# osqp/OSQP.jl

Hardware: AMD Instinct MI355X
Metric: ADMM iterations/sec (higher is better)
Workload: dtype f64; 1 GPU; rand-1e6; n=1000000, m=1000000, nnz_A=1000000000, nnz_P_full=1000749500, nnz_P_triu=500874750, backend=pcg, check_termination=25, adaptive_rho_interval=50, instances=1

## Files before the change

### osqp.jl_amd/csrc/common.hpp

```cpp
#pragma once
#include <chrono>
#include <hip/hip_runtime.h>
#include <cstdint>
#include <cstdio>
#include <cstdlib>
#include <cstring>
#include <stdexcept>
#include <string>
#include <vector>

#include "../../include/osqp_amd.h"

namespace oq {

struct Error : std::runtime_error {
  int code;
  Error(int c, const std::string &m) : std::runtime_error(m), code(c) {}
};
struct PanelRefused : Error {
  using Error::Error;
};
struct UnsortedColumns : Error {
  UnsortedColumns() : Error(1, "the row indices inside a column of A must ascend (and not repeat)") {}
};
extern thread_local bool g_unsorted_columns;
struct TreeFault : Error {
  TreeFault() : Error(6, "internal: a supernode of the triangular solve waited 200 ms for its children (the solves fall back to one launch per level)") {}
};
void set_last_error(const std::string &m);

#define HIP_CHECK(expr)                                                                             \
  do {                                                                                              \
    hipError_t _e = (expr);                                                                         \
    if (_e != hipSuccess)                                                                           \
      throw oq::Error(6, std::string("HIP error: ") + hipGetErrorString(_e) + " at " + __FILE__ +   \
                             ":" + std::to_string(__LINE__));                                       \
  } while (0)

extern int g_debug_sync;
inline void post_launch(const char *name, hipStream_t s) {
  hipError_t e = hipGetLastError();
  if (e != hipSuccess) throw Error(6, std::string("launch of ") + name + " failed: " + hipGetErrorString(e));
  if (g_debug_sync) {
    fprintf(stderr, "[osqp-amd] %s ... ", name);
    fflush(stderr);
    e = hipStreamSynchronize(s);
    fprintf(stderr, "%s\n", e == hipSuccess ? "ok" : hipGetErrorString(e));
    if (e != hipSuccess) throw Error(6, std::string("kernel ") + name + " failed: " + hipGetErrorString(e));
  }
}
#define OQ_LAUNCH(kern, grid, block, shmem, stream, ...)                    \
  do {                                                                      \
    hipLaunchKernelGGL(kern, grid, block, shmem, stream, __VA_ARGS__);      \
    oq::post_launch(#kern, stream);                                         \
  } while (0)

extern size_t g_device_bytes;
extern size_t g_device_peak;
extern double g_alloc_s, g_free_s;
extern size_t g_cache_bytes;
inline double wall_now() { return std::chrono::duration<double>(std::chrono::steady_clock::now().time_since_epoch()).count(); }

size_t dev_size_class(size_t bytes);
void *dev_alloc(size_t bytes, size_t &granted);
void dev_free(void *p, size_t granted);
void dev_cache_trim();
size_t dev_va_reserved();
struct DevCacheScope {
  DevCacheScope();
  ~DevCacheScope();
  DevCacheScope(const DevCacheScope &) = delete;
  DevCacheScope &operator=(const DevCacheScope &) = delete;
};

template <typename T>
struct DevBuf {
  T *p = nullptr;
  size_t n = 0;
  size_t cap = 0;
  DevBuf() = default;
  explicit DevBuf(size_t count) { alloc(count); }
  DevBuf(const DevBuf &) = delete;
  DevBuf &operator=(const DevBuf &) = delete;
  DevBuf(DevBuf &&o) noexcept : p(o.p), n(o.n), cap(o.cap) { o.p = nullptr; o.n = 0; o.cap = 0; }
  DevBuf &operator=(DevBuf &&o) noexcept {
    if (this != &o) { release(); p = o.p; n = o.n; cap = o.cap; o.p = nullptr; o.n = 0; o.cap = 0; }
    return *this;
  }
  ~DevBuf() { release(); }
  void alloc(size_t count) {
    release();
    n = count;
    p = (T *)dev_alloc((count ? count : 1) * sizeof(T), cap);
  }
  void release() {
    if (p) {
      dev_free(p, cap);
      p = nullptr;
      n = 0;
      cap = 0;
    }
  }
  void zero(hipStream_t s) { HIP_CHECK(hipMemsetAsync(p, 0, (n ? n : 1) * sizeof(T), s)); }
  void upload(const T *h, size_t count, hipStream_t s) {
    if (count) HIP_CHECK(hipMemcpyAsync(p, h, count * sizeof(T), hipMemcpyHostToDevice, s));
  }
  void download(T *h, size_t count, hipStream_t s) const {
    if (count) HIP_CHECK(hipMemcpyAsync(h, p, count * sizeof(T), hipMemcpyDeviceToHost, s));
  }
  T *get() const { return p; }
};

struct DevPanel {
  bool active = false;
  int W = 0, shift = 0, B = 0, Gp = 1, NG = 0, ntiles = 0;
  DevBuf<int> tile_g, tile_r0, tile_r1;
  DevBuf<int> unit_s0, unit_ns;
  DevBuf<uint32_t> slice_base;
  DevBuf<int> slice_len;
  DevBuf<int> slice_rows;
  DevBuf<uint32_t> cellbase;
  DevBuf<double> sval;
  DevBuf<uint16_t> scol;
  bool wide = false;
  DevBuf<uint32_t> scol32;
  DevBuf<double> partial;
  size_t padded = 0;
};

struct DevCsr {
  int rows = 0, cols = 0;
  int64_t nnz = 0;
  DevBuf<int64_t> rowptr;
  DevBuf<int> col;
  DevBuf<double> val;
  DevPanel panel;
  bool compact = false;
  int group = 64;
  double spmv_bytes() const {
    return 12.0 * (double)nnz + 4.0 * ((double)rows + 1.0) + 8.0 * ((double)rows + (double)cols);
  }
};

enum Slot {
  S_PRI = 0, S_PRI_UNS, S_Z, S_AX, S_Z_UNS, S_AX_UNS,
  S_DUA, S_DUA_UNS, S_Q, S_ATY, S_PX, S_Q_UNS, S_ATY_UNS, S_PX_UNS,
  S_XPX, S_QX,
  S_T0, S_T1, S_T2, S_T3, S_T4, S_T5,
  S_COUNT = 32
};

struct Publish {
  double *host_slots = nullptr;
  volatile unsigned long long *host_seq = nullptr;
  unsigned long long seq = 0;
};

constexpr int kBlock = 256;
constexpr int kReduceBlocks = 1024;

inline int blocks_for(int64_t n, int per_block = kBlock) {
  int64_t b = (n + per_block - 1) / per_block;
  if (b < 1) b = 1;
  if (b > 2147483647LL) throw Error(6, "grid too large");
  return (int)b;
}

}
```

### osqp.jl_amd/csrc/panel.hip

```cpp
#include <algorithm>

#include "kernels.hpp"
#include <functional>
#include "devutil.hpp"

namespace oq {

namespace {

constexpr int kThreads = 1024;
#ifndef OQ_SELL_BATCH
#define OQ_SELL_BATCH 16
#endif
constexpr int kBatch = OQ_SELL_BATCH;
constexpr int kWaves = kThreads / 64;
constexpr int kTileRowsMax = 3968;
constexpr int kSortN = 4096;

int env_int(const char *name, int dflt) { const char *e = getenv(name); return e ? atoi(e) : dflt; }
int panel_shift() { return env_int("OSQP_AMD_PANEL_SHIFT", 14); }
int panel_tile_nnz() { return env_int("OSQP_AMD_PANEL_TILE_NNZ", 65536); }

__device__ __forceinline__ int64_t lower_bound_col(const int *__restrict__ col, int64_t s, int64_t e, int target) {
  while (s < e) { int64_t mid = (s + e) >> 1; if (col[mid] < target) s = mid + 1; else e = mid; }
  return s;
}

__global__ __launch_bounds__(kBlock) void k_panel_count(int rows, int B, int shift, const int64_t *__restrict__ rp,
                                                        const int *__restrict__ col, int64_t *__restrict__ cnt,
                                                        uint32_t *__restrict__ cellsrc) {
  const int lane = threadIdx.x & 63;
  const int64_t row = ((int64_t)blockIdx.x * kBlock + threadIdx.x) >> 6;
  if (row >= rows) return;
  const int64_t s = rp[row], e = rp[row + 1];
  for (int b = lane; b < B; b += 64) {
    int64_t lo = lower_bound_col(col, s, e, b << shift);
    int64_t hi = (b + 1 == B) ? e : lower_bound_col(col, s, e, (b + 1) << shift);
    cnt[(size_t)b * rows + row] = hi - lo;
    cellsrc[(size_t)b * rows + row] = (uint32_t)lo;
  }
}

__global__ __launch_bounds__(kBlock) void k_group_count(int rows, int B, int Gp, int64_t gcells, const int64_t *__restrict__ cnt,
                                                        int64_t *__restrict__ gcnt) {
  const int64_t c = (int64_t)blockIdx.x * kBlock + threadIdx.x;
  if (c >= gcells) return;
  const int64_t g = c / rows;
  const int r = (int)(c - g * rows);
  int64_t a = 0;
  for (int b = (int)g * Gp; b < B && b < ((int)g + 1) * Gp; b++) a += cnt[(size_t)b * rows + r];
  gcnt[c] = a;
}
__global__ __launch_bounds__(kBlock) void k_expand_units(int ntiles, int B, int Gp, const int *__restrict__ tile_g,
                                                         const int *__restrict__ tile_r0, const int *__restrict__ tile_r1,
                                                         int *__restrict__ ub, int *__restrict__ u0, int *__restrict__ u1) {
  const int64_t u = (int64_t)blockIdx.x * kBlock + threadIdx.x;
  if (u >= (int64_t)ntiles * Gp) return;
  const int t = (int)(u / Gp), j = (int)(u - (int64_t)t * Gp);
  const int b = tile_g[t] * Gp + j;
  const bool real = b < B;
  ub[u] = real ? b : 0;
  u0[u] = tile_r0[t];
  u1[u] = real ? tile_r1[t] : tile_r0[t];
}

__global__ __launch_bounds__(kBlock) void k_tile_cost(int64_t cells, int64_t cmin, int64_t *__restrict__ cnt) {
  const int64_t c = (int64_t)blockIdx.x * kBlock + threadIdx.x;
  if (c < cells && cnt[c] < cmin) cnt[c] = cmin;
}
__global__ __launch_bounds__(kBlock) void k_tile_starts(int rows, int64_t cells, const int64_t *__restrict__ coff, int64_t budget,
                                                        int64_t *__restrict__ start) {
  const int64_t c = (int64_t)blockIdx.x * kBlock + threadIdx.x;
  if (c >= cells) return;
  const int64_t b = c / rows;
  const int r = (int)(c - b * rows);
  const int64_t *po = coff + b * rows;
  const int64_t base = po[0];
  start[c] = (r == 0 || (po[r - 1] - base) / budget != (po[r] - base) / budget) ? 1 : 0;
}
__global__ __launch_bounds__(kBlock) void k_tile_fill(int rows, int64_t cells, const int64_t *__restrict__ start,
                                                      const int64_t *__restrict__ tid, int *__restrict__ tile_b, int *__restrict__ tile_r0) {
  const int64_t c = (int64_t)blockIdx.x * kBlock + threadIdx.x;
  if (c >= cells || !start[c]) return;
  const int64_t b = c / rows;
  tile_b[tid[c]] = (int)b;
  tile_r0[tid[c]] = (int)(c - b * rows);
}
__global__ __launch_bounds__(kBlock) void k_tile_ends(int rows, int ntiles, const int *__restrict__ tile_b, const int *__restrict__ tile_r0,
                                                      int *__restrict__ tile_r1) {
  const int t = blockIdx.x * kBlock + threadIdx.x;
  if (t >= ntiles) return;
  tile_r1[t] = (t + 1 < ntiles && tile_b[t + 1] == tile_b[t]) ? tile_r0[t + 1] : rows;
}

__device__ void order_tile_rows(uint32_t *key, const int64_t *__restrict__ po, int r0, int nrows, int *nz_rows) {
  if (threadIdx.x == 0) *nz_rows = 0;
  __syncthreads();
  int mine = 0;
  for (int i = threadIdx.x; i < kSortN; i += kThreads) {
    uint32_t k = 0xFFFFFFFFu;
    if (i < nrows) {
      const uint32_t len = (uint32_t)(po[r0 + i + 1] - po[r0 + i]);
      k = ((0x7FFFFu - len) << 12) | (uint32_t)i;
      mine += len > 0;
    }
    key[i] = k;
  }
  if (mine) atomicAdd(nz_rows, mine);
  __syncthreads();
  for (int k = 2; k <= kSortN; k <<= 1)
    for (int j = k >> 1; j > 0; j >>= 1) {
      for (int i = threadIdx.x; i < kSortN; i += kThreads) {
        const int p = i ^ j;
        if (p > i) {
          const uint32_t a = key[i], b = key[p];
          if ((a > b) == ((i & k) == 0)) { key[i] = b; key[p] = a; }
        }
      }
      __syncthreads();
    }
}
__device__ __forceinline__ uint32_t key_len(uint32_t key) { return 0x7FFFFu - (key >> 12); }

__global__ __launch_bounds__(kThreads) void k_tile_measure(int rows, const int *__restrict__ tile_b, const int *__restrict__ tile_r0,
                                                           const int *__restrict__ tile_r1, const int64_t *__restrict__ off,
                                                           int64_t *__restrict__ nslices, int64_t *__restrict__ padded) {
  __shared__ uint32_t key[kSortN];
  __shared__ int nz;
  __shared__ unsigned long long total;
  const int t = blockIdx.x;
  const int r0 = tile_r0[t], nrows = tile_r1[t] - r0;
  if (threadIdx.x == 0) total = 0ULL;
  order_tile_rows(key, off + (size_t)tile_b[t] * rows, r0, nrows, &nz);
  const int ns = (nz + 63) >> 6;
  unsigned long long mine = 0;
  for (int sl = threadIdx.x; sl < ns; sl += kThreads) mine += 64ULL * key_len(key[sl * 64]);
  if (mine) atomicAdd(&total, mine);
  __syncthreads();
  if (threadIdx.x == 0) { nslices[t] = ns; padded[t] = (int64_t)total; }
}
__global__ __launch_bounds__(kThreads) void k_tile_layout(int rows, const int *__restrict__ tile_b, const int *__restrict__ tile_r0,
                                                          const int *__restrict__ tile_r1, const int64_t *__restrict__ off,
                                                          const int64_t *__restrict__ slice0, const int64_t *__restrict__ padded0,
                                                          int *__restrict__ tile_s0, int *__restrict__ tile_ns,
                                                          uint32_t *__restrict__ slice_base, int *__restrict__ slice_len,
                                                          int *__restrict__ slice_rows, uint32_t *__restrict__ cellbase) {
  __shared__ uint32_t key[kSortN];
  __shared__ uint32_t sbase[kSortN / 64 + 1];
  __shared__ int nz;
  const int t = blockIdx.x, b = tile_b[t];
  const int r0 = tile_r0[t], nrows = tile_r1[t] - r0;
  order_tile_rows(key, off + (size_t)b * rows, r0, nrows, &nz);
  const int ns = (nz + 63) >> 6;
  if (threadIdx.x == 0) {
    uint32_t acc = (uint32_t)padded0[t];
    for (int sl = 0; sl < ns; sl++) { sbase[sl] = acc; acc += 64u * key_len(key[sl * 64]); }
    tile_s0[t] = (int)slice0[t];
    tile_ns[t] = ns;
  }
  __syncthreads();
  const int64_t s0 = slice0[t];
  for (int i = threadIdx.x; i < ns * 64; i += kThreads) {
    const int sl = i >> 6, lane = i & 63;
    int row = -1;
    if (i < nz) {
      row = r0 + (int)(key[i] & 4095u);
      cellbase[(size_t)b * rows + row] = sbase[sl] + (uint32_t)lane;
    }
    slice_rows[(size_t)(s0 + sl) * 64 + lane] = row;
    if (lane == 0) { slice_base[s0 + sl] = sbase[sl]; slice_len[s0 + sl] = (int)key_len(key[sl * 64]); }
  }
}

template <typename ColT>
__global__ __launch_bounds__(kBlock) void k_sell_scatter(int rows, int shift, const int64_t *__restrict__ rp, const int *__restrict__ col,
                                                         const double *__restrict__ val, const uint32_t *__restrict__ cellbase,
                                                         ColT *__restrict__ scol, double *__restrict__ sval, int with_cols,
                                                         uint32_t *__restrict__ slot) {
  const int lane = threadIdx.x & 63;
  const int64_t row = ((int64_t)blockIdx.x * kBlock + threadIdx.x) >> 6;
  if (row >= rows) return;
  const int64_t s = rp[row], e = rp[row + 1];
  const int mask = (1 << shift) - 1;
  int carry_b = -1;
  int64_t carry_seg = s;
  for (int64_t k0 = s; k0 < e; k0 += 64) {
    const int64_t k = k0 + lane;
    const bool in = k < e;
    const int c = in ? col[k] : 0x7fffffff;
    const int b = in ? (c >> shift) : 0x7fffffff;
    int bprev = __shfl_up(b, 1, 64);
    if (lane == 0) bprev = carry_b;
    const unsigned long long heads = __ballot(b != bprev);
    const unsigned long long upto = heads & (~0ull >> (63 - lane));
    const int64_t seg = upto ? k0 + (63 - __builtin_clzll(upto)) : carry_seg;
    if (in) {
      const size_t dst = (size_t)cellbase[(size_t)b * rows + row] + (size_t)(k - seg) * 64;
      sval[dst] = val[k];
      if (with_cols) scol[dst] = (ColT)(c & mask);
      if (slot) slot[k] = (uint32_t)dst;
    }
    carry_b = __shfl(b, 63, 64);
    carry_seg = __shfl(seg, 63, 64);
  }
}

constexpr int kFillK = 16;
constexpr int kFillStride = 65;
constexpr int kFillWaves = 4;
template <typename ColT>
__global__ __launch_bounds__(kFillWaves * 64) void k_sell_fill_lds(int rows, int shift, const int *__restrict__ ub, const int *__restrict__ unit_s0,
                                                                 const int *__restrict__ unit_ns, const uint32_t *__restrict__ slice_base,
                                                                 const int *__restrict__ slice_len, const int *__restrict__ slice_rows,
                                                                 const uint32_t *__restrict__ cellsrc, const int64_t *__restrict__ off,
                                                                 const int *__restrict__ col, const double *__restrict__ val,
                                                                 ColT *__restrict__ scol, double *__restrict__ sval, uint32_t *__restrict__ slot,
                                                                 int what) {
  const bool do_cols = what & 1, do_vals = what & 2;
  __shared__ double tv[kFillWaves][kFillK * kFillStride];
  __shared__ uint32_t tc[kFillWaves][kFillK * kFillStride];
  __shared__ int start[kFillWaves][65];
  const int u = blockIdx.x, b = ub[u];
  const int s0 = unit_s0[u], ns = unit_ns[u];
  const int wave = threadIdx.x >> 6, lane = threadIdx.x & 63;
  const int mask = (1 << shift) - 1;
  double *mv = tv[wave];
  uint32_t *mc = tc[wave];
  int *st = start[wave];
  for (int sl = s0 + wave; sl < s0 + ns; sl += kFillWaves) {
    const uint32_t base = slice_base[sl];
    const int L = slice_len[sl];
    const int row = slice_rows[(size_t)sl * 64 + lane];
    uint32_t src = 0;
    int len = 0;
    if (row >= 0) {
      const size_t c = (size_t)b * rows + row;
      src = cellsrc[c];
      len = (int)(off[c + 1] - off[c]);
    }
    for (int k0 = 0; k0 < L; k0 += kFillK) {
      int mine = len - k0;
      mine = mine < 0 ? 0 : (mine > kFillK ? kFillK : mine);
      int incl = mine;
#pragma unroll
      for (int o = 1; o < 64; o <<= 1) { const int t = __shfl_up(incl, o, 64); if (lane >= o) incl += t; }
      const int total = __shfl(incl, 63, 64);
      st[lane] = incl - mine;
      if (lane == 63) st[64] = total;
      __builtin_amdgcn_fence(__ATOMIC_RELEASE, "wavefront");
      __builtin_amdgcn_wave_barrier();
      __builtin_amdgcn_fence(__ATOMIC_ACQUIRE, "wavefront");
      for (int f = lane; f < ((total + 63) & ~63); f += 64) {
        const bool in = f < total;
        int r = 0;
        if (in) {
          int lo = 0, hi = 64;
          while (hi - lo > 1) { const int mid = (lo + hi) >> 1; if (st[mid] <= f) lo = mid; else hi = mid; }
          r = lo;
        }
        const uint32_t rsrc = (uint32_t)__shfl((int)src, r, 64);
        if (in) {
          const int k = f - st[r];
          const size_t g = (size_t)rsrc + (size_t)(k0 + k);
          if (do_vals) mv[k * kFillStride + r] = val[g];
          if (do_cols) {
            mc[k * kFillStride + r] = (uint32_t)(col[g] & mask);
            if (slot) slot[g] = base + (uint32_t)((k0 + k) * 64 + r);
          }
        }
      }
      __builtin_amdgcn_fence(__ATOMIC_RELEASE, "wavefront");
      __builtin_amdgcn_wave_barrier();
      __builtin_amdgcn_fence(__ATOMIC_ACQUIRE, "wavefront");
      const int kend = L - k0 < kFillK ? L - k0 : kFillK;
      for (int k = 0; k < kend; k++) {
        const size_t at = (size_t)base + (size_t)(k0 + k) * 64 + lane;
        const bool in = k < mine;
        if (do_vals) sval[at] = in ? mv[k * kFillStride + lane] : 0.0;
        if (do_cols) scol[at] = in ? (ColT)mc[k * kFillStride + lane] : (ColT)0;
      }
      __builtin_amdgcn_fence(__ATOMIC_RELEASE, "wavefront");
      __builtin_amdgcn_wave_barrier();
    }
  }
}

template <typename ColT, bool kStageX, bool kSquare>
__device__ __forceinline__ void sell_tile(int t, int rows, int cols, int shift, int B, int Gp, const int *__restrict__ tile_g,
                                          const int *__restrict__ tile_r0, const int *__restrict__ tile_r1,
                                          const int *__restrict__ unit_s0, const int *__restrict__ unit_ns,
                                          const uint32_t *__restrict__ slice_base, const int *__restrict__ slice_len,
                                          const int *__restrict__ slice_rows, const ColT *__restrict__ scol,
                                          const double *__restrict__ sval, const double *__restrict__ x, double *__restrict__ partial) {
  extern __shared__ __attribute__((aligned(16))) double lds[];
  const int g = tile_g[t];
  const int W = 1 << shift;
  const int r0 = tile_r0[t], nrows = tile_r1[t] - r0;
  double *xs_lds = lds;
  double *ys = kStageX ? lds + W : lds;
  for (int i = threadIdx.x; i < nrows; i += kThreads) ys[i] = 0.0;
  const int wave = threadIdx.x >> 6, lane = threadIdx.x & 63;
  bool first = true;
  for (int j = 0; j < Gp; j++) {
    const int b = g * Gp + j;
    if (b >= B) break;
    const int s0 = unit_s0[(size_t)t * Gp + j], ns = unit_ns[(size_t)t * Gp + j];
    if (ns == 0) continue;
    const int c0 = b << shift;
    const double *xs = x + c0;
    if (kStageX) {
      if (!first) __syncthreads();
      const int wlen = cols - c0 < W ? cols - c0 : W;
      double2 *xl = reinterpret_cast<double2 *>(xs_lds);
      if (wlen == 16 * kThreads) {
        const double2 *xg = reinterpret_cast<const double2 *>(x + c0);
        double2 v[8];
#pragma unroll
        for (int k = 0; k < 8; k++) v[k] = xg[threadIdx.x + k * kThreads];
#pragma unroll
        for (int k = 0; k < 8; k++) xl[threadIdx.x + k * kThreads] = v[k];
      } else {
        for (int i = threadIdx.x; i < wlen; i += kThreads) xs_lds[i] = x[c0 + i];
      }
      __syncthreads();
      xs = xs_lds;
    } else {
      __syncthreads();
    }
    first = false;
    int sl = s0 + wave;
    size_t nbase = 0;
    int nL = 0, nrow = -1;
    if (sl < s0 + ns) { nbase = (size_t)slice_base[sl]; nL = slice_len[sl]; nrow = slice_rows[(size_t)sl * 64 + lane]; }
    for (; sl < s0 + ns; sl += kWaves) {
      const size_t base = nbase + lane;
      const int L = nL, row = nrow;
      if (sl + kWaves < s0 + ns) {
        nbase = (size_t)slice_base[sl + kWaves]; nL = slice_len[sl + kWaves]; nrow = slice_rows[(size_t)(sl + kWaves) * 64 + lane];
      }
      const double *v = sval + base;
      const ColT *c = scol + base;
      double a0 = 0.0;
      for (int k = 0; k < L; k += kBatch) {
        double cv[kBatch];
        ColT cc[kBatch];
        if (k + kBatch <= L) {
#pragma unroll
          for (int u = 0; u < kBatch; u++) { cv[u] = v[(size_t)(k + u) * 64]; cc[u] = c[(size_t)(k + u) * 64]; }
        } else {
#pragma unroll
          for (int u = 0; u < kBatch; u++) {
            const bool in = k + u < L;
            cv[u] = in ? v[(size_t)(k + u) * 64] : 0.0;
            cc[u] = in ? c[(size_t)(k + u) * 64] : (ColT)0;
          }
        }
#pragma unroll
        for (int u = 0; u < kBatch; u++) a0 += (kSquare ? cv[u] * cv[u] : cv[u]) * xs[cc[u]];
      }
      if (row >= 0) ys[row - r0] += a0;
    }
  }
  __syncthreads();
  double *out = partial + (size_t)g * rows + r0;
  for (int i = threadIdx.x; i < nrows; i += kThreads) out[i] = ys[i];
}
template <typename ColT, bool kStageX, bool kSquare = false>
__global__ __launch_bounds__(kThreads) void k_spmv_sell(int rows, int cols, int shift, int B, int Gp, const int *__restrict__ tile_g,
                                                        const int *__restrict__ tile_r0, const int *__restrict__ tile_r1,
                                                        const int *__restrict__ unit_s0, const int *__restrict__ unit_ns,
                                                        const uint32_t *__restrict__ slice_base, const int *__restrict__ slice_len,
                                                        const int *__restrict__ slice_rows, const ColT *__restrict__ scol,
                                                        const double *__restrict__ sval, const double *__restrict__ x,
                                                        double *__restrict__ partial, const int *__restrict__ skip) {
  if (skip && *skip) return;
  sell_tile<ColT, kStageX, kSquare>(blockIdx.x, rows, cols, shift, B, Gp, tile_g, tile_r0, tile_r1, unit_s0, unit_ns, slice_base, slice_len,
                                    slice_rows, scol, sval, x, partial);
}
struct SellSide {
  int rows, cols, B, Gp, ntiles;
  const int *tile_g, *tile_r0, *tile_r1, *unit_s0, *unit_ns, *slice_len, *slice_rows;
  const uint32_t *slice_base;
  const uint16_t *scol;
  const double *sval;
  double *partial;
};
__global__ __launch_bounds__(kThreads) void k_spmv_sell_pair(SellSide a, SellSide b, int shift, const double *__restrict__ x,
                                                             const int *__restrict__ skip) {
  if (skip && *skip) return;
  const bool first = (int)blockIdx.x < a.ntiles;
  const SellSide &m = first ? a : b;
  sell_tile<uint16_t, true, false>(first ? (int)blockIdx.x : (int)blockIdx.x - a.ntiles, m.rows, m.cols, shift, m.B, m.Gp, m.tile_g, m.tile_r0,
                                   m.tile_r1, m.unit_s0, m.unit_ns, m.slice_base, m.slice_len, m.slice_rows, m.scol, m.sval, x, m.partial);
}

__device__ __forceinline__ void panel_reduce_rows(int vb, int vg, int rows, int B, const double *__restrict__ partial, double *__restrict__ y,
                                                  const double *__restrict__ rscale, double beta, double gamma,
                                                  const double *__restrict__ v, const SpmvExtra &ex) {
  double dot = 0.0, mx = 0.0, num = 0.0, den = 0.0;
  for (int i = vb * kBlock + threadIdx.x; i < rows; i += vg * kBlock) {
    double acc = 0.0;
    int b = 0;
    for (; b + 8 <= B; b += 8) {
      double t[8];
#pragma unroll
      for (int u = 0; u < 8; u++) t[u] = partial[(size_t)(b + u) * rows + i];
#pragma unroll
      for (int u = 0; u < 8; u++) acc += t[u];
    }
    if (b + 4 <= B) {
      double t[4];
#pragma unroll
      for (int u = 0; u < 4; u++) t[u] = partial[(size_t)(b + u) * rows + i];
#pragma unroll
      for (int u = 0; u < 4; u++) acc += t[u];
      b += 4;
    }
    for (; b < B; b++) acc += partial[(size_t)b * rows + i];
    if (ex.y2) ex.y2[i] = ex.s2[i] * acc;
    if (rscale) acc *= rscale[i];
    if (beta != 0.0) acc += beta * y[i];
    if (v) acc += gamma * v[i];
    y[i] = acc;
    if (ex.dotv) dot += ex.dotv[i] * acc;
    if (ex.absmax_slot) mx = nanmax(mx, fabs(acc));
    if (ex.e2_partials) {
      const double d = ex.e2_x1[i] - ex.e2_x0[i], m1 = ex.e2_m1[i];
      num += d * (acc - m1);
      den += d * (m1 - ex.e2_m0[i]);
    }
  }
  if (ex.e2_partials) {
    num = block_sum(num);
    den = block_sum(den);
    if (threadIdx.x == 0) { ex.e2_partials[vb] = num; ex.e2_partials[kReduceBlocks + vb] = den; }
    if (vb == 0)
      for (int t = vg + threadIdx.x; t < kReduceBlocks; t += kBlock) { ex.e2_partials[t] = 0.0; ex.e2_partials[kReduceBlocks + t] = 0.0; }
  }
  if (ex.dot_partials) {
    dot = block_sum(dot);
    if (threadIdx.x == 0) ex.dot_partials[vb] = dot;
    if (vb == 0)
      for (int t = vg + threadIdx.x; t < kReduceBlocks; t += kBlock) ex.dot_partials[t] = 0.0;
  }
  if (ex.absmax_slot) {
    mx = block_max(mx);
    if (threadIdx.x == 0) atomic_max_nonneg(ex.absmax_slot, mx);
  }
}
__global__ __launch_bounds__(kBlock) void k_panel_reduce(int rows, int B, const double *__restrict__ partial, double *__restrict__ y,
                                                         const double *__restrict__ rscale, double beta, double gamma,
                                                         const double *__restrict__ v, SpmvExtra ex, const int *__restrict__ skip) {
  if (skip && *skip) return;
  panel_reduce_rows(blockIdx.x, gridDim.x, rows, B, partial, y, rscale, beta, gamma, v, ex);
}
struct ReduceSide {
  int rows, B, grid;
  const double *partial;
  double *y;
  double gamma;
  const double *v;
  SpmvExtra ex;
};
__global__ __launch_bounds__(kBlock) void k_panel_reduce_pair(ReduceSide a, ReduceSide b, const int *__restrict__ skip) {
  if (skip && *skip) return;
  const bool first = (int)blockIdx.x < a.grid;
  const ReduceSide &m = first ? a : b;
  panel_reduce_rows(first ? (int)blockIdx.x : (int)blockIdx.x - a.grid, m.grid, m.rows, m.B, m.partial, m.y, nullptr, 0.0, m.gamma, m.v, m.ex);
}

template <typename ColT, int kOp>
__global__ __launch_bounds__(kThreads) void k_sell_visit(int rows, int shift, int B, int Gp, const int *__restrict__ tile_g,
                                                         const int *__restrict__ tile_r0, const int *__restrict__ tile_r1,
                                                         const int *__restrict__ unit_s0, const int *__restrict__ unit_ns,
                                                         const uint32_t *__restrict__ slice_base, const int *__restrict__ slice_len,
                                                         const int *__restrict__ slice_rows, const ColT *__restrict__ scol,
                                                         double *__restrict__ sval, const double *__restrict__ r, const double *__restrict__ c,
                                                         int order, double scalar, int row0, double *__restrict__ out) {
  __shared__ double ys[kOp == 1 ? kTileRowsMax : 1];
  const int t = blockIdx.x, g = tile_g[t];
  const int r0 = tile_r0[t], nrows = tile_r1[t] - r0;
  const int wave = threadIdx.x >> 6, lane = threadIdx.x & 63;
  if (kOp == 1) for (int i = threadIdx.x; i < nrows; i += kThreads) ys[i] = 0.0;
  for (int j = 0; j < Gp; j++) {
    const int b = g * Gp + j;
    if (b >= B) break;
    const int s0 = unit_s0[(size_t)t * Gp + j], ns = unit_ns[(size_t)t * Gp + j];
    if (kOp == 1) __syncthreads();
    const int c0 = b << shift;
    for (int sl = s0 + wave; sl < s0 + ns; sl += kWaves) {
      const size_t base = (size_t)slice_base[sl] + lane;
      const int L = slice_len[sl];
      const int row = slice_rows[(size_t)sl * 64 + lane];
      if (row < 0) continue;
      double mx = 0.0;
      for (int k = 0; k < L; k++) {
        const size_t at = base + (size_t)k * 64;
        double v = sval[at];
        if (kOp == 0) {
          if (r) {
            const int col = c0 + (int)scol[at];
            double a, bb;
            if (order == 1) { const int gi = row + row0; const int lo = col < gi ? col : gi, hi = col < gi ? gi : col; a = c[lo]; bb = c[hi]; }
            else if (order == 2) { a = c[col]; bb = r[row]; }
            else { a = r[row]; bb = c[col]; }
            v = (v * a) * bb;
          }
          if (scalar != 1.0) v *= scalar;
          if (v != 0.0 || sval[at] != 0.0) sval[at] = v;
        } else if (kOp == 1) {
          mx = fmax(mx, fabs(v));
        } else {
          if (c0 + (int)scol[at] == row + row0 && v != 0.0) out[row] = v;
        }
      }
      if (kOp == 1) ys[row - r0] = fmax(ys[row - r0], mx);
    }
  }
  if (kOp == 1) {
    __syncthreads();
    double *o = out + (size_t)g * rows + r0;
    for (int i = threadIdx.x; i < nrows; i += kThreads) o[i] = ys[i];
  }
}
template <typename ColT>
__global__ __launch_bounds__(kThreads) void k_sell_scale_norm(int rows, int cols, int shift, int B, int Gp, const int *__restrict__ tile_g,
                                                              const int *__restrict__ tile_r0, const int *__restrict__ tile_r1,
                                                              const int *__restrict__ unit_s0, const int *__restrict__ unit_ns,
                                                              const uint32_t *__restrict__ slice_base, const int *__restrict__ slice_len,
                                                              const int *__restrict__ slice_rows, const ColT *__restrict__ scol,
                                                              double *__restrict__ sval, const double *__restrict__ r,
                                                              const double *__restrict__ c, int order, double pre, int row0,
                                                              double *__restrict__ partial) {
  extern __shared__ __attribute__((aligned(16))) double lds[];
  const int t = blockIdx.x, g = tile_g[t];
  const int W = 1 << shift;
  const int r0 = tile_r0[t], nrows = tile_r1[t] - r0;
  double *cs = lds, *ys = lds + W;
  for (int i = threadIdx.x; i < nrows; i += kThreads) ys[i] = 0.0;
  const int wave = threadIdx.x >> 6, lane = threadIdx.x & 63;
  const double *rv = order == 1 ? c + row0 : r;
  bool first = true;
  for (int j = 0; j < Gp; j++) {
    const int b = g * Gp + j;
    if (b >= B) break;
    const int s0 = unit_s0[(size_t)t * Gp + j], ns = unit_ns[(size_t)t * Gp + j];
    if (ns == 0) continue;
    const int c0 = b << shift;
    if (!first) __syncthreads();
    const int wlen = cols - c0 < W ? cols - c0 : W;
    if (wlen == 16 * kThreads) {
      const double2 *xg = reinterpret_cast<const double2 *>(c + c0);
      double2 *xl = reinterpret_cast<double2 *>(cs);
      double2 v[8];
#pragma unroll
      for (int k = 0; k < 8; k++) v[k] = xg[threadIdx.x + k * kThreads];
#pragma unroll
      for (int k = 0; k < 8; k++) xl[threadIdx.x + k * kThreads] = v[k];
    } else {
      for (int i = threadIdx.x; i < wlen; i += kThreads) cs[i] = c[c0 + i];
    }
    __syncthreads();
    first = false;
    int sl = s0 + wave;
    size_t nbase = 0;
    int nL = 0, nrow = -1;
    double nrs = 1.0;
    if (sl < s0 + ns) {
      nbase = (size_t)slice_base[sl]; nL = slice_len[sl]; nrow = slice_rows[(size_t)sl * 64 + lane];
      nrs = nrow >= 0 ? rv[nrow] : 1.0;
    }
    for (; sl < s0 + ns; sl += kWaves) {
      const size_t base = nbase + lane;
      const int L = nL, row = nrow;
      const double rs = nrs;
      if (sl + kWaves < s0 + ns) {
        nbase = (size_t)slice_base[sl + kWaves]; nL = slice_len[sl + kWaves]; nrow = slice_rows[(size_t)(sl + kWaves) * 64 + lane];
        nrs = nrow >= 0 ? rv[nrow] : 1.0;
      }
      double *v = sval + base;
      const ColT *cc_ = scol + base;
      const int grow = row + row0 - c0;
      double mx = 0.0;
      for (int k = 0; k < L; k += kBatch) {
        double cv[kBatch];
        ColT cc[kBatch];
        const bool full = k + kBatch <= L;
        if (full) {
#pragma unroll
          for (int u = 0; u < kBatch; u++) { cv[u] = v[(size_t)(k + u) * 64]; cc[u] = cc_[(size_t)(k + u) * 64]; }
        } else {
#pragma unroll
          for (int u = 0; u < kBatch; u++) {
            const bool in = k + u < L;
            cv[u] = in ? v[(size_t)(k + u) * 64] : 0.0;
            cc[u] = in ? cc_[(size_t)(k + u) * 64] : (ColT)0;
          }
        }
#pragma unroll
        for (int u = 0; u < kBatch; u++) {
          double x = cv[u];
          if (pre != 1.0) x *= pre;
          const double cf = cs[cc[u]];
          if (order == 1) { const bool below = (int)cc[u] < grow; x = (x * (below ? cf : rs)) * (below ? rs : cf); }
          else if (order == 2) x = (x * cf) * rs;
          else x = (x * rs) * cf;
          cv[u] = x;
          mx = fmax(mx, fabs(x));
        }
        if (row >= 0) {
          if (full) {
#pragma unroll
            for (int u = 0; u < kBatch; u++) v[(size_t)(k + u) * 64] = cv[u];
          } else {
#pragma unroll
            for (int u = 0; u < kBatch; u++) if (k + u < L) v[(size_t)(k + u) * 64] = cv[u];
          }
        }
      }
      if (row >= 0) ys[row - r0] = fmax(ys[row - r0], mx);
    }
  }
  __syncthreads();
  double *out = partial + (size_t)g * rows + r0;
  for (int i = threadIdx.x; i < nrows; i += kThreads) out[i] = ys[i];
}
__global__ __launch_bounds__(kBlock) void k_panel_reduce_max(int rows, int NG, const double *__restrict__ partial, double *__restrict__ out,
                                                             int accumulate) {
  const int i = blockIdx.x * kBlock + threadIdx.x;
  if (i >= rows) return;
  double m = 0.0;
  for (int g = 0; g < NG; g++) m = fmax(m, partial[(size_t)g * rows + i]);
  out[i] = accumulate ? fmax(out[i], m) : m;
}
__global__ __launch_bounds__(kBlock) void k_sell_slot_of_pos(int rows, int shift, const int64_t *__restrict__ rp, const int *__restrict__ col,
                                                             const uint32_t *__restrict__ cellbase, uint32_t *__restrict__ slot) {
  const int lane = threadIdx.x & 63;
  const int64_t row = ((int64_t)blockIdx.x * kBlock + threadIdx.x) >> 6;
  if (row >= rows) return;
  const int64_t s = rp[row], e = rp[row + 1];
  for (int64_t k = s + lane; k < e; k += 64) {
    const int b = col[k] >> shift;
    const int64_t seg = lower_bound_col(col, s, k + 1, b << shift);
    slot[k] = (uint32_t)((size_t)cellbase[(size_t)b * rows + row] + (size_t)(k - seg) * 64);
  }
}

size_t spmv_lds_bytes(int shift) { return (sizeof(double) << shift) + sizeof(double) * kTileRowsMax; }

int64_t read_i64(const int64_t *dev, hipStream_t s) {
  int64_t v = 0;
  HIP_CHECK(hipMemcpyAsync(&v, dev, sizeof(int64_t), hipMemcpyDeviceToHost, s));
  HIP_CHECK(hipStreamSynchronize(s));
  return v;
}

}

static int panel_group_size(const DevCsr &M, int B) {
  const int want = env_int("OSQP_AMD_PANEL_GROUP", 0);
  if (want > 0) return std::min(want, B);
  if ((double)M.nnz / (4.0 * (double)panel_tile_nnz()) >= 1024.0) return std::min(4, B);
  return 1;
}

static int wide_shift(const DevCsr &M) {
  if (const int forced = env_int("OSQP_AMD_WIDE_SHIFT", 0)) return forced;
  for (int sh = 18; sh <= 20; sh++) {
    const int Bw = (M.cols + (1 << sh) - 1) >> sh;
    if (Bw < 4) return 0;
    if ((double)M.nnz / ((double)M.rows * Bw) >= 3.5) return sh;
  }
  return 0;
}
static int panel_mode(const DevCsr &M) {
  const int shift = panel_shift();
  if (const char *e = getenv("OSQP_AMD_PANEL")) {
    if (atoi(e) == 0) return 0;
    if (atoi(e) == 2) return M.cols > (1 << shift) ? 1 : 0;
    if (atoi(e) == 3) return M.cols > (1 << shift) ? 2 : 0;
  }
  if (M.nnz < 2000000 || M.nnz >= 4000000000LL) return 0;
  const int B = (M.cols + (1 << shift) - 1) >> shift;
  if (B >= 2) {
    const int Gp = panel_group_size(M, B), NG = (B + Gp - 1) / Gp;
    if ((double)M.nnz / ((double)M.rows * NG) >= 4.0 && (double)M.nnz / ((double)M.rows * B) >= 1.5) return 1;
  }
  return wide_shift(M) ? 2 : 0;
}

bool panel_wanted(const DevCsr &M) { return panel_mode(M) != 0; }

void panel_fill(DevCsr &M, bool with_cols, hipStream_t s, uint32_t *slot) {
  DevPanel &P = M.panel;
  if (P.wide)
    OQ_LAUNCH(k_sell_scatter<uint32_t>, dim3(blocks_for((int64_t)M.rows * 64)), dim3(kBlock), 0, s, M.rows, P.shift, M.rowptr.get(),
              M.col.get(), M.val.get(), P.cellbase.get(), P.scol32.get(), P.sval.get(), with_cols ? 1 : 0, slot);
  else
    OQ_LAUNCH(k_sell_scatter<uint16_t>, dim3(blocks_for((int64_t)M.rows * 64)), dim3(kBlock), 0, s, M.rows, P.shift, M.rowptr.get(),
              M.col.get(), M.val.get(), P.cellbase.get(), P.scol.get(), P.sval.get(), with_cols ? 1 : 0, slot);
}

void panel_build(DevCsr &M, hipStream_t s, uint32_t *slot, bool will_compact, const std::function<void()> &after_cols) {
  DevPanel &P = M.panel;
  P.wide = panel_mode(M) == 2;
  P.shift = P.wide ? (wide_shift(M) ? wide_shift(M) : 18) : panel_shift(); P.W = 1 << P.shift;
  if (!P.wide && P.shift > 15) throw PanelRefused(6, "panel width above 2^15 columns is not supported (16-bit local column ids, LDS size)");
  P.B = (M.cols + P.W - 1) >> P.shift;
  const int64_t cells = (int64_t)P.B * M.rows;
  DevBuf<int64_t> cnt((size_t)cells + 1), off((size_t)cells + 1);
  DevBuf<uint32_t> cellsrc((size_t)cells);
  OQ_LAUNCH(k_panel_count, dim3(blocks_for((int64_t)M.rows * 64)), dim3(kBlock), 0, s, M.rows, P.B, P.shift, M.rowptr.get(),
            M.col.get(), cnt.get(), cellsrc.get());
  exclusive_scan(cnt.get(), off.get(), cells, s);
  P.Gp = panel_group_size(M, P.B);
  P.NG = (P.B + P.Gp - 1) / P.Gp;
  const int64_t gcells = (int64_t)P.NG * M.rows;
  DevBuf<int64_t> gcnt((size_t)gcells + 1), tid((size_t)gcells + 1);
  OQ_LAUNCH(k_group_count, dim3(blocks_for(gcells)), dim3(kBlock), 0, s, M.rows, P.B, P.Gp, gcells, cnt.get(), gcnt.get());
  cnt.release();
  int64_t tile_nnz = panel_tile_nnz();
  if (!getenv("OSQP_AMD_PANEL_TILE_NNZ") && P.Gp == 1) {
    int dev = 0, cus = 256;
    if (hipGetDevice(&dev) == hipSuccess) (void)hipDeviceGetAttribute(&cus, hipDeviceAttributeMultiprocessorCount, dev);
    if ((double)M.nnz / (double)tile_nnz < (double)cus)
      tile_nnz = std::max<int64_t>(32768, std::min<int64_t>(tile_nnz, (int64_t)((double)M.nnz / (0.85 * (double)cus))));
  }
  const int64_t budget = std::max<int64_t>(tile_nnz * P.Gp, kTileRowsMax);
  const int64_t cmin = (budget + kTileRowsMax - 1) / kTileRowsMax;
  OQ_LAUNCH(k_tile_cost, dim3(blocks_for(gcells)), dim3(kBlock), 0, s, gcells, cmin, gcnt.get());
  exclusive_scan(gcnt.get(), tid.get(), gcells, s);
  OQ_LAUNCH(k_tile_starts, dim3(blocks_for(gcells)), dim3(kBlock), 0, s, M.rows, gcells, tid.get(), budget, gcnt.get());
  exclusive_scan(gcnt.get(), tid.get(), gcells, s);
  const int64_t ntiles = read_i64(tid.get() + gcells, s);
  if (ntiles <= 0 || ntiles * P.Gp >= 2147483647LL) throw PanelRefused(6, "panel layout: bad tile count");
  P.ntiles = (int)ntiles;
  P.tile_g.alloc((size_t)ntiles); P.tile_r0.alloc((size_t)ntiles); P.tile_r1.alloc((size_t)ntiles);
  OQ_LAUNCH(k_tile_fill, dim3(blocks_for(gcells)), dim3(kBlock), 0, s, M.rows, gcells, gcnt.get(), tid.get(), P.tile_g.get(), P.tile_r0.get());
  OQ_LAUNCH(k_tile_ends, dim3(blocks_for(ntiles)), dim3(kBlock), 0, s, M.rows, P.ntiles, P.tile_g.get(), P.tile_r0.get(), P.tile_r1.get());
  const int64_t nunits = ntiles * P.Gp;
  DevBuf<int> ub((size_t)nunits), u0((size_t)nunits), u1((size_t)nunits);
  OQ_LAUNCH(k_expand_units, dim3(blocks_for(nunits)), dim3(kBlock), 0, s, P.ntiles, P.B, P.Gp, P.tile_g.get(), P.tile_r0.get(),
            P.tile_r1.get(), ub.get(), u0.get(), u1.get());
  HIP_CHECK(hipStreamSynchronize(s));
  gcnt.release(); tid.release();
  DevBuf<int64_t> nsl((size_t)nunits + 1), pad((size_t)nunits + 1), slice0((size_t)nunits + 1), padded0((size_t)nunits + 1);
  OQ_LAUNCH(k_tile_measure, dim3((unsigned)nunits), dim3(kThreads), 0, s, M.rows, ub.get(), u0.get(), u1.get(), off.get(), nsl.get(), pad.get());
  exclusive_scan(nsl.get(), slice0.get(), nunits, s);
  exclusive_scan(pad.get(), padded0.get(), nunits, s);
  const int64_t nslices = read_i64(slice0.get() + nunits, s), padded = read_i64(padded0.get() + nunits, s);
  if (padded >= 4294967295LL) throw PanelRefused(6, "sliced-ELL copy exceeds 2^32 entries");
  if (!getenv("OSQP_AMD_PANEL") && (double)padded > 1.5 * (double)M.nnz) throw PanelRefused(6, "sliced-ELL copy would be mostly padding");
  P.padded = (size_t)padded;
  P.unit_s0.alloc((size_t)nunits); P.unit_ns.alloc((size_t)nunits);
  P.slice_base.alloc((size_t)nslices); P.slice_len.alloc((size_t)nslices); P.slice_rows.alloc((size_t)nslices * 64);
  P.cellbase.alloc((size_t)cells); P.cellbase.zero(s);
  OQ_LAUNCH(k_tile_layout, dim3((unsigned)nunits), dim3(kThreads), 0, s, M.rows, ub.get(), u0.get(), u1.get(), off.get(), slice0.get(),
            padded0.get(), P.unit_s0.get(), P.unit_ns.get(), P.slice_base.get(), P.slice_len.get(), P.slice_rows.get(), P.cellbase.get());
  P.partial.alloc((size_t)gcells);
  P.partial.zero(s);
  static const bool lds_fill = !(getenv("OSQP_AMD_SELL_FILL") && atoi(getenv("OSQP_AMD_SELL_FILL")) == 0);
  auto fill = [&](int what) {
    if (P.wide)
      OQ_LAUNCH(k_sell_fill_lds<uint32_t>, dim3((unsigned)nunits), dim3(kFillWaves * 64), 0, s, M.rows, P.shift, ub.get(), P.unit_s0.get(),
                P.unit_ns.get(), P.slice_base.get(), P.slice_len.get(), P.slice_rows.get(), cellsrc.get(), off.get(), M.col.get(), M.val.get(),
                P.scol32.get(), P.sval.get(), slot, what);
    else
      OQ_LAUNCH(k_sell_fill_lds<uint16_t>, dim3((unsigned)nunits), dim3(kFillWaves * 64), 0, s, M.rows, P.shift, ub.get(), P.unit_s0.get(),
                P.unit_ns.get(), P.slice_base.get(), P.slice_len.get(), P.slice_rows.get(), cellsrc.get(), off.get(), M.col.get(), M.val.get(),
                P.scol.get(), P.sval.get(), slot, what);
  };
  if (!lds_fill) {
    P.sval.alloc((size_t)padded);
    P.sval.zero(s);
    if (P.wide) { P.scol32.alloc((size_t)padded); P.scol32.zero(s); }
    else { P.scol.alloc((size_t)padded); P.scol.zero(s); }
    panel_fill(M, true, s, slot);
  } else if (will_compact && !P.wide) {
    P.scol.alloc((size_t)padded);
    fill(1);
    HIP_CHECK(hipStreamSynchronize(s));
    M.col.release();
    if (after_cols) after_cols();
    P.sval.alloc((size_t)padded);
    fill(2);
  } else {
    P.sval.alloc((size_t)padded);
    if (P.wide) P.scol32.alloc((size_t)padded); else P.scol.alloc((size_t)padded);
    fill(3);
  }
  HIP_CHECK(hipStreamSynchronize(s));
  if (!P.wide)
    HIP_CHECK(hipFuncSetAttribute((const void *)k_spmv_sell<uint16_t, true>, hipFuncAttributeMaxDynamicSharedMemorySize,
                                  (int)spmv_lds_bytes(P.shift)));
  P.active = true;
}

static int reduce_grid(int rows) { return std::min(blocks_for(rows), kReduceBlocks); }

void spmv_panel(const DevCsr &M, const double *x, double *y, const double *rscale, double beta, double gamma, const double *v,
                hipStream_t s, const SpmvExtra *extra) {
  const DevPanel &P = M.panel;
  const SpmvExtra ex = extra ? *extra : SpmvExtra();
  if (P.wide)
    OQ_LAUNCH((k_spmv_sell<uint32_t, false>), dim3(P.ntiles), dim3(kThreads), sizeof(double) * kTileRowsMax, s, M.rows, M.cols, P.shift, P.B,
              P.Gp, P.tile_g.get(), P.tile_r0.get(), P.tile_r1.get(), P.unit_s0.get(), P.unit_ns.get(), P.slice_base.get(),
              P.slice_len.get(), P.slice_rows.get(), P.scol32.get(), P.sval.get(), x, P.partial.get(), g_skip);
  else
    OQ_LAUNCH((k_spmv_sell<uint16_t, true>), dim3(P.ntiles), dim3(kThreads), spmv_lds_bytes(P.shift), s, M.rows, M.cols, P.shift, P.B,
              P.Gp, P.tile_g.get(), P.tile_r0.get(), P.tile_r1.get(), P.unit_s0.get(), P.unit_ns.get(), P.slice_base.get(),
              P.slice_len.get(), P.slice_rows.get(), P.scol.get(), P.sval.get(), x, P.partial.get(), g_skip);
  OQ_LAUNCH(k_panel_reduce, dim3(reduce_grid(M.rows)), dim3(kBlock), 0, s, M.rows, P.NG, P.partial.get(), y, rscale, beta, gamma, v, ex, g_skip);
}

bool spmv_pair_ok(const DevCsr &Ma, const DevCsr &Mb) {
  const DevPanel &A = Ma.panel, &B = Mb.panel;
  static const bool enabled = !(getenv("OSQP_AMD_SPMV_PAIR") && atoi(getenv("OSQP_AMD_SPMV_PAIR")) == 0);
  return enabled && A.active && B.active && !A.wide && !B.wide && A.shift == B.shift && Ma.cols == Mb.cols && A.ntiles + B.ntiles <= 2048;
}
void spmv_pair(const DevCsr &Ma, const DevCsr &Mb, const double *x, double *ya, const SpmvExtra *extra_a, double *yb, double gamma_b,
               const double *vb, hipStream_t s) {
  auto side = [](const DevCsr &M) {
    const DevPanel &P = M.panel;
    SellSide t;
    t.rows = M.rows; t.cols = M.cols; t.B = P.B; t.Gp = P.Gp; t.ntiles = P.ntiles;
    t.tile_g = P.tile_g.get(); t.tile_r0 = P.tile_r0.get(); t.tile_r1 = P.tile_r1.get(); t.unit_s0 = P.unit_s0.get(); t.unit_ns = P.unit_ns.get();
    t.slice_len = P.slice_len.get(); t.slice_rows = P.slice_rows.get(); t.slice_base = P.slice_base.get(); t.scol = P.scol.get();
    t.sval = P.sval.get(); t.partial = P.partial.get();
    return t;
  };
  const DevPanel &A = Ma.panel, &B = Mb.panel;
  static bool attr_set = false;
  if (!attr_set) {
    HIP_CHECK(hipFuncSetAttribute((const void *)k_spmv_sell_pair, hipFuncAttributeMaxDynamicSharedMemorySize, (int)spmv_lds_bytes(A.shift)));
    attr_set = true;
  }
  OQ_LAUNCH(k_spmv_sell_pair, dim3(A.ntiles + B.ntiles), dim3(kThreads), spmv_lds_bytes(A.shift), s, side(Ma), side(Mb), A.shift, x, g_skip);
  ReduceSide ra{Ma.rows, A.NG, reduce_grid(Ma.rows), A.partial.get(), ya, 0.0, nullptr, extra_a ? *extra_a : SpmvExtra()};
  ReduceSide rb{Mb.rows, B.NG, reduce_grid(Mb.rows), B.partial.get(), yb, gamma_b, vb, SpmvExtra()};
  OQ_LAUNCH(k_panel_reduce_pair, dim3(ra.grid + rb.grid), dim3(kBlock), 0, s, ra, rb, g_skip);
}

#define OQ_SELL_VISIT(OP, ...)                                                                                                              \
  do {                                                                                                                                      \
    if (P.wide) OQ_LAUNCH((k_sell_visit<uint32_t, OP>), dim3(P.ntiles), dim3(kThreads), 0, s, M.rows, P.shift, P.B, P.Gp, P.tile_g.get(),    \
                          P.tile_r0.get(), P.tile_r1.get(), P.unit_s0.get(), P.unit_ns.get(), P.slice_base.get(), P.slice_len.get(),        \
                          P.slice_rows.get(), P.scol32.get(), P.sval.get(), __VA_ARGS__);                                                    \
    else OQ_LAUNCH((k_sell_visit<uint16_t, OP>), dim3(P.ntiles), dim3(kThreads), 0, s, M.rows, P.shift, P.B, P.Gp, P.tile_g.get(),           \
                   P.tile_r0.get(), P.tile_r1.get(), P.unit_s0.get(), P.unit_ns.get(), P.slice_base.get(), P.slice_len.get(),               \
                   P.slice_rows.get(), P.scol.get(), P.sval.get(), __VA_ARGS__);                                                             \
  } while (0)

void panel_row_absmax(const DevCsr &M, double *out, bool accumulate, hipStream_t s) {
  const DevPanel &P = M.panel;
  OQ_SELL_VISIT(1, (const double *)nullptr, (const double *)nullptr, 0, 1.0, 0, P.partial.get());
  OQ_LAUNCH(k_panel_reduce_max, dim3(blocks_for(M.rows)), dim3(kBlock), 0, s, M.rows, P.NG, P.partial.get(), out, (int)accumulate);
}
void panel_scale(DevCsr &M, const double *r, const double *c, int order, double scalar, hipStream_t s, int row0) {
  const DevPanel &P = M.panel;
  OQ_SELL_VISIT(0, r, c, order, scalar, row0, (double *)nullptr);
}
void panel_scale_norm(DevCsr &M, const double *r, const double *c, int order, double pre, int row0, double *norm, hipStream_t s) {
  const DevPanel &P = M.panel;
  if (P.wide) throw Error(6, "internal: the fused scaling pass needs LDS-staged panels");
  HIP_CHECK(hipFuncSetAttribute((const void *)k_sell_scale_norm<uint16_t>, hipFuncAttributeMaxDynamicSharedMemorySize,
                                (int)spmv_lds_bytes(P.shift)));
  OQ_LAUNCH((k_sell_scale_norm<uint16_t>), dim3(P.ntiles), dim3(kThreads), spmv_lds_bytes(P.shift), s, M.rows, M.cols, P.shift, P.B, P.Gp,
            P.tile_g.get(), P.tile_r0.get(), P.tile_r1.get(), P.unit_s0.get(), P.unit_ns.get(), P.slice_base.get(), P.slice_len.get(),
            P.slice_rows.get(), P.scol.get(), P.sval.get(), r, c, order, pre, row0, P.partial.get());
  OQ_LAUNCH(k_panel_reduce_max, dim3(blocks_for(M.rows)), dim3(kBlock), 0, s, M.rows, P.NG, P.partial.get(), norm, 0);
}
void panel_diag(const DevCsr &M, double *diag, int row0, hipStream_t s) {
  const DevPanel &P = M.panel;
  HIP_CHECK(hipMemsetAsync(diag, 0, sizeof(double) * (size_t)M.rows, s));
  OQ_SELL_VISIT(2, (const double *)nullptr, (const double *)nullptr, 0, 1.0, row0, diag);
}
#undef OQ_SELL_VISIT
void spmv_panel_squared(const DevCsr &M, const double *x, double *y, double gamma, const double *v, hipStream_t s) {
  const DevPanel &P = M.panel;
  HIP_CHECK(hipFuncSetAttribute((const void *)k_spmv_sell<uint16_t, true, true>, hipFuncAttributeMaxDynamicSharedMemorySize,
                                (int)spmv_lds_bytes(P.shift)));
  OQ_LAUNCH((k_spmv_sell<uint16_t, true, true>), dim3(P.ntiles), dim3(kThreads), spmv_lds_bytes(P.shift), s, M.rows, M.cols, P.shift, P.B,
            P.Gp, P.tile_g.get(), P.tile_r0.get(), P.tile_r1.get(), P.unit_s0.get(), P.unit_ns.get(), P.slice_base.get(),
            P.slice_len.get(), P.slice_rows.get(), P.scol.get(), P.sval.get(), x, P.partial.get(), (const int *)nullptr);
  OQ_LAUNCH(k_panel_reduce, dim3(reduce_grid(M.rows)), dim3(kBlock), 0, s, M.rows, P.NG, P.partial.get(), y, (const double *)nullptr, 0.0, gamma, v,
            SpmvExtra(), (const int *)nullptr);
}
void panel_slot_of_pos(const DevCsr &M, uint32_t *slot, hipStream_t s) {
  const DevPanel &P = M.panel;
  OQ_LAUNCH(k_sell_slot_of_pos, dim3(blocks_for((int64_t)M.rows * 64)), dim3(kBlock), 0, s, M.rows, P.shift, M.rowptr.get(), M.col.get(),
            P.cellbase.get(), slot);
}
bool panel_can_compact(const DevCsr &M) { return M.panel.active && !M.panel.wide; }
void panel_compact(DevCsr &M) {
  M.col.release();
  M.val.release();
  M.panel.cellbase.release();
  M.compact = true;
}

}
```

Baseline: 83.39 iterations/s.

## Compact SELL slices by dropping padding lanes per column in aligned groups

Changes the SELL panel layout so that each column of a slice only stores as many lanes as the rows still active there, rounded up to an alignment group (default 64, set through an env var). It packs row length and local row index into one per-lane word, adds per-slice column-start tables, and updates the measure, layout, scatter, fill and SpMV kernels to compute offsets with ballot/popcount. The aim is to cut padded zero storage and memory traffic in SpMV for rows of uneven length. In exchange it adds per-element offset arithmetic, less regular access patterns and extra setup tables.

```diff
diff --git a/osqp.jl_amd/csrc/common.hpp b/osqp.jl_amd/csrc/common.hpp
--- a/osqp.jl_amd/csrc/common.hpp
+++ b/osqp.jl_amd/csrc/common.hpp
@@ -118,8 +118,10 @@
   DevBuf<int> unit_s0, unit_ns;
   DevBuf<uint32_t> slice_base;
   DevBuf<int> slice_len;
-  DevBuf<int> slice_rows;
+  DevBuf<uint32_t> slice_lanes;
+  int align = 64;
   DevBuf<uint32_t> cellbase;
+  DevBuf<uint32_t> slice_tab, colstart;
   DevBuf<double> sval;
   DevBuf<uint16_t> scol;
   bool wide = false;
diff --git a/osqp.jl_amd/csrc/panel.hip b/osqp.jl_amd/csrc/panel.hip
--- a/osqp.jl_amd/csrc/panel.hip
+++ b/osqp.jl_amd/csrc/panel.hip
@@ -2,6 +2,7 @@
 
 #include "kernels.hpp"
 #include <functional>
+#include <type_traits>
 #include "devutil.hpp"
 
 namespace oq {
@@ -20,6 +21,12 @@
 int env_int(const char *name, int dflt) { const char *e = getenv(name); return e ? atoi(e) : dflt; }
 int panel_shift() { return env_int("OSQP_AMD_PANEL_SHIFT", 14); }
 int panel_tile_nnz() { return env_int("OSQP_AMD_PANEL_TILE_NNZ", 65536); }
+constexpr int kSellAlign = 64;
+constexpr int kSlack = 64;
+int sell_align() {
+  const int g = env_int("OSQP_AMD_SELL_ALIGN", kSellAlign);
+  return (g >= 1 && g <= 64 && (g & (g - 1)) == 0) ? g : kSellAlign;
+}
 
 __device__ __forceinline__ int64_t lower_bound_col(const int *__restrict__ col, int64_t s, int64_t e, int target) {
   while (s < e) { int64_t mid = (s + e) >> 1; if (col[mid] < target) s = mid + 1; else e = mid; }
@@ -121,60 +128,99 @@
     }
 }
 __device__ __forceinline__ uint32_t key_len(uint32_t key) { return 0x7FFFFu - (key >> 12); }
-
-__global__ __launch_bounds__(kThreads) void k_tile_measure(int rows, const int *__restrict__ tile_b, const int *__restrict__ tile_r0,
+__device__ __forceinline__ int lane_len(uint32_t w) { return (int)(w >> 12); }
+__device__ __forceinline__ int lane_row(uint32_t w, int r0) { return w ? r0 + (int)(w & 4095u) : -1; }
+template <typename T>
+__device__ __forceinline__ T &slice_at(T *base, uint32_t idx) {
+  return *reinterpret_cast<T *>(reinterpret_cast<char *>(const_cast<typename std::remove_const<T>::type *>(base)) + (size_t)(idx * (uint32_t)sizeof(T)));
+}
+__device__ __forceinline__ int wave_id() { return __builtin_amdgcn_readfirstlane((int)(threadIdx.x >> 6)); }
+__device__ __forceinline__ uint32_t column_lanes(bool in, int gm) {
+  return (uint32_t)((__popcll(__ballot(in)) + gm) & ~gm);
+}
+
+__global__ __launch_bounds__(kThreads) void k_tile_measure(int rows, int G, const int *__restrict__ tile_b, const int *__restrict__ tile_r0,
                                                            const int *__restrict__ tile_r1, const int64_t *__restrict__ off,
-                                                           int64_t *__restrict__ nslices, int64_t *__restrict__ padded) {
+                                                           int64_t *__restrict__ nslices, int64_t *__restrict__ padded,
+                                                           int64_t *__restrict__ lensum) {
   __shared__ uint32_t key[kSortN];
   __shared__ int nz;
-  __shared__ unsigned long long total;
+  __shared__ unsigned long long total, total64;
   const int t = blockIdx.x;
   const int r0 = tile_r0[t], nrows = tile_r1[t] - r0;
-  if (threadIdx.x == 0) total = 0ULL;
+  if (threadIdx.x == 0) { total = 0ULL; total64 = 0ULL; }
   order_tile_rows(key, off + (size_t)tile_b[t] * rows, r0, nrows, &nz);
   const int ns = (nz + 63) >> 6;
-  unsigned long long mine = 0;
-  for (int sl = threadIdx.x; sl < ns; sl += kThreads) mine += 64ULL * key_len(key[sl * 64]);
+  unsigned long long mine = 0, mine64 = 0;
+  for (int i = threadIdx.x * G; i < nz; i += kThreads * G) {
+    mine += (unsigned long long)G * key_len(key[i]);
+    if ((i & 63) == 0) mine64 += key_len(key[i]);
+  }
   if (mine) atomicAdd(&total, mine);
+  if (mine64) atomicAdd(&total64, mine64);
   __syncthreads();
-  if (threadIdx.x == 0) { nslices[t] = ns; padded[t] = (int64_t)total; }
-}
-__global__ __launch_bounds__(kThreads) void k_tile_layout(int rows, const int *__restrict__ tile_b, const int *__restrict__ tile_r0,
+  if (threadIdx.x == 0) { nslices[t] = ns; padded[t] = (int64_t)total; lensum[t] = (int64_t)total64; }
+}
+__global__ __launch_bounds__(kThreads) void k_tile_layout(int rows, int G, const int *__restrict__ tile_b, const int *__restrict__ tile_r0,
                                                           const int *__restrict__ tile_r1, const int64_t *__restrict__ off,
                                                           const int64_t *__restrict__ slice0, const int64_t *__restrict__ padded0,
-                                                          int *__restrict__ tile_s0, int *__restrict__ tile_ns,
-                                                          uint32_t *__restrict__ slice_base, int *__restrict__ slice_len,
-                                                          int *__restrict__ slice_rows, uint32_t *__restrict__ cellbase) {
+                                                          const int64_t *__restrict__ lensum0, int *__restrict__ tile_s0,
+                                                          int *__restrict__ tile_ns, uint32_t *__restrict__ slice_base,
+                                                          int *__restrict__ slice_len, uint32_t *__restrict__ slice_lanes,
+                                                          uint32_t *__restrict__ cellbase, uint32_t *__restrict__ slice_tab,
+                                                          uint32_t *__restrict__ colstart) {
   __shared__ uint32_t key[kSortN];
-  __shared__ uint32_t sbase[kSortN / 64 + 1];
+  __shared__ uint32_t sbase[kSortN / 64 + 1], stab[kSortN / 64 + 1];
   __shared__ int nz;
   const int t = blockIdx.x, b = tile_b[t];
   const int r0 = tile_r0[t], nrows = tile_r1[t] - r0;
+  for (int i = threadIdx.x; i <= kSortN / 64; i += kThreads) sbase[i] = 0u;
   order_tile_rows(key, off + (size_t)b * rows, r0, nrows, &nz);
   const int ns = (nz + 63) >> 6;
+  for (int i = threadIdx.x * G; i < nz; i += kThreads * G) atomicAdd(&sbase[i >> 6], (uint32_t)G * key_len(key[i]));
+  __syncthreads();
   if (threadIdx.x == 0) {
-    uint32_t acc = (uint32_t)padded0[t];
-    for (int sl = 0; sl < ns; sl++) { sbase[sl] = acc; acc += 64u * key_len(key[sl * 64]); }
+    uint32_t acc = (uint32_t)padded0[t], tab = (uint32_t)lensum0[t];
+    for (int sl = 0; sl < ns; sl++) {
+      const uint32_t size = sbase[sl];
+      sbase[sl] = acc; acc += size;
+      stab[sl] = tab; tab += key_len(key[sl * 64]);
+    }
     tile_s0[t] = (int)slice0[t];
     tile_ns[t] = ns;
   }
   __syncthreads();
   const int64_t s0 = slice0[t];
+  const int gm = G - 1;
   for (int i = threadIdx.x; i < ns * 64; i += kThreads) {
     const int sl = i >> 6, lane = i & 63;
-    int row = -1;
+    uint32_t w = 0u;
     if (i < nz) {
-      row = r0 + (int)(key[i] & 4095u);
-      cellbase[(size_t)b * rows + row] = sbase[sl] + (uint32_t)lane;
-    }
-    slice_rows[(size_t)(s0 + sl) * 64 + lane] = row;
-    if (lane == 0) { slice_base[s0 + sl] = sbase[sl]; slice_len[s0 + sl] = (int)key_len(key[sl * 64]); }
-  }
-}
-
+      const uint32_t local = key[i] & 4095u;
+      w = (key_len(key[i]) << 12) | local;
+      cellbase[(size_t)b * rows + r0 + (int)local] = (uint32_t)(s0 + sl) * 64u + (uint32_t)lane;
+    }
+    slice_lanes[(size_t)(s0 + sl) * 64 + lane] = w;
+    const int len = lane_len(w), L = (int)key_len(key[sl * 64]);
+    if (lane == 0) { slice_base[s0 + sl] = sbase[sl]; slice_len[s0 + sl] = L; slice_tab[s0 + sl] = stab[sl]; }
+    uint32_t start = 0u;
+    for (int k = 0; k < L; k++) {
+      if (lane == 0) colstart[(size_t)stab[sl] + k] = start;
+      start += column_lanes(k < len, gm);
+    }
+  }
+}
+
+__device__ __forceinline__ size_t cell_slot(uint32_t cell, int64_t j, const uint32_t *__restrict__ slice_base,
+                                            const uint32_t *__restrict__ slice_tab, const uint32_t *__restrict__ colstart) {
+  const uint32_t sl = cell >> 6;
+  return (size_t)slice_base[sl] + (size_t)colstart[(size_t)slice_tab[sl] + (size_t)j] + (size_t)(cell & 63u);
+}
 template <typename ColT>
 __global__ __launch_bounds__(kBlock) void k_sell_scatter(int rows, int shift, const int64_t *__restrict__ rp, const int *__restrict__ col,
                                                          const double *__restrict__ val, const uint32_t *__restrict__ cellbase,
+                                                         const uint32_t *__restrict__ slice_base, const uint32_t *__restrict__ slice_tab,
+                                                         const uint32_t *__restrict__ colstart,
                                                          ColT *__restrict__ scol, double *__restrict__ sval, int with_cols,
                                                          uint32_t *__restrict__ slot) {
   const int lane = threadIdx.x & 63;
@@ -195,7 +241,7 @@
     const unsigned long long upto = heads & (~0ull >> (63 - lane));
     const int64_t seg = upto ? k0 + (63 - __builtin_clzll(upto)) : carry_seg;
     if (in) {
-      const size_t dst = (size_t)cellbase[(size_t)b * rows + row] + (size_t)(k - seg) * 64;
+      const size_t dst = cell_slot(cellbase[(size_t)b * rows + row], k - seg, slice_base, slice_tab, colstart);
       sval[dst] = val[k];
       if (with_cols) scol[dst] = (ColT)(c & mask);
       if (slot) slot[k] = (uint32_t)dst;
@@ -209,10 +255,11 @@
 constexpr int kFillStride = 65;
 constexpr int kFillWaves = 4;
 template <typename ColT>
-__global__ __launch_bounds__(kFillWaves * 64) void k_sell_fill_lds(int rows, int shift, const int *__restrict__ ub, const int *__restrict__ unit_s0,
+__global__ __launch_bounds__(kFillWaves * 64) void k_sell_fill_lds(int rows, int shift, int gm, const int *__restrict__ ub, const int *__restrict__ u0,
+                                                                 const int *__restrict__ unit_s0,
                                                                  const int *__restrict__ unit_ns, const uint32_t *__restrict__ slice_base,
-                                                                 const int *__restrict__ slice_len, const int *__restrict__ slice_rows,
-                                                                 const uint32_t *__restrict__ cellsrc, const int64_t *__restrict__ off,
+                                                                 const int *__restrict__ slice_len, const uint32_t *__restrict__ slice_lanes,
+                                                                 const uint32_t *__restrict__ cellsrc,
                                                                  const int *__restrict__ col, const double *__restrict__ val,
                                                                  ColT *__restrict__ scol, double *__restrict__ sval, uint32_t *__restrict__ slot,
                                                                  int what) {
@@ -220,7 +267,7 @@
   __shared__ double tv[kFillWaves][kFillK * kFillStride];
   __shared__ uint32_t tc[kFillWaves][kFillK * kFillStride];
   __shared__ int start[kFillWaves][65];
-  const int u = blockIdx.x, b = ub[u];
+  const int u = blockIdx.x, b = ub[u], r0 = u0[u];
   const int s0 = unit_s0[u], ns = unit_ns[u];
   const int wave = threadIdx.x >> 6, lane = threadIdx.x & 63;
   const int mask = (1 << shift) - 1;
@@ -230,17 +277,18 @@
   for (int sl = s0 + wave; sl < s0 + ns; sl += kFillWaves) {
     const uint32_t base = slice_base[sl];
     const int L = slice_len[sl];
-    const int row = slice_rows[(size_t)sl * 64 + lane];
-    uint32_t src = 0;
-    int len = 0;
-    if (row >= 0) {
-      const size_t c = (size_t)b * rows + row;
-      src = cellsrc[c];
-      len = (int)(off[c + 1] - off[c]);
-    }
+    const uint32_t w = slice_lanes[(size_t)sl * 64 + lane];
+    const int row = lane_row(w, r0), len = lane_len(w);
+    const uint32_t src = row >= 0 ? cellsrc[(size_t)b * rows + row] : 0u;
+    uint32_t cstart = 0u;
     for (int k0 = 0; k0 < L; k0 += kFillK) {
       int mine = len - k0;
       mine = mine < 0 ? 0 : (mine > kFillK ? kFillK : mine);
+      uint32_t kstart = 0u;
+      for (int k = 0; k < kFillK; k++) {
+        if (lane == k) kstart = cstart;
+        cstart += column_lanes(k < mine, gm);
+      }
       int incl = mine;
 #pragma unroll
       for (int o = 1; o < 64; o <<= 1) { const int t = __shfl_up(incl, o, 64); if (lane >= o) incl += t; }
@@ -263,21 +311,22 @@
           const int k = f - st[r];
           const size_t g = (size_t)rsrc + (size_t)(k0 + k);
           if (do_vals) mv[k * kFillStride + r] = val[g];
-          if (do_cols) {
-            mc[k * kFillStride + r] = (uint32_t)(col[g] & mask);
-            if (slot) slot[g] = base + (uint32_t)((k0 + k) * 64 + r);
-          }
+          if (do_cols) mc[k * kFillStride + r] = (uint32_t)(col[g] & mask);
         }
+        const uint32_t ks = (uint32_t)__shfl((int)kstart, in ? f - st[r] : 0, 64);
+        if (in && do_cols && slot) slot[(size_t)rsrc + (size_t)(k0 + f - st[r])] = base + ks + (uint32_t)r;
       }
       __builtin_amdgcn_fence(__ATOMIC_RELEASE, "wavefront");
       __builtin_amdgcn_wave_barrier();
       __builtin_amdgcn_fence(__ATOMIC_ACQUIRE, "wavefront");
       const int kend = L - k0 < kFillK ? L - k0 : kFillK;
       for (int k = 0; k < kend; k++) {
-        const size_t at = (size_t)base + (size_t)(k0 + k) * 64 + lane;
+        const size_t at = (size_t)base + (size_t)__shfl((int)kstart, k, 64) + lane;
         const bool in = k < mine;
-        if (do_vals) sval[at] = in ? mv[k * kFillStride + lane] : 0.0;
-        if (do_cols) scol[at] = in ? (ColT)mc[k * kFillStride + lane] : (ColT)0;
+        if (lane < (int)column_lanes(in, gm)) {
+          if (do_vals) sval[at] = in ? mv[k * kFillStride + lane] : 0.0;
+          if (do_cols) scol[at] = in ? (ColT)mc[k * kFillStride + lane] : (ColT)0;
+        }
       }
       __builtin_amdgcn_fence(__ATOMIC_RELEASE, "wavefront");
       __builtin_amdgcn_wave_barrier();
@@ -286,11 +335,11 @@
 }
 
 template <typename ColT, bool kStageX, bool kSquare>
-__device__ __forceinline__ void sell_tile(int t, int rows, int cols, int shift, int B, int Gp, const int *__restrict__ tile_g,
+__device__ __forceinline__ void sell_tile(int t, int rows, int cols, int shift, int gm, int B, int Gp, const int *__restrict__ tile_g,
                                           const int *__restrict__ tile_r0, const int *__restrict__ tile_r1,
                                           const int *__restrict__ unit_s0, const int *__restrict__ unit_ns,
                                           const uint32_t *__restrict__ slice_base, const int *__restrict__ slice_len,
-                                          const int *__restrict__ slice_rows, const ColT *__restrict__ scol,
+                                          const uint32_t *__restrict__ slice_lanes, const ColT *__restrict__ scol,
                                           const double *__restrict__ sval, const double *__restrict__ x, double *__restrict__ partial) {
   extern __shared__ __attribute__((aligned(16))) double lds[];
   const int g = tile_g[t];
@@ -299,7 +348,7 @@
   double *xs_lds = lds;
   double *ys = kStageX ? lds + W : lds;
   for (int i = threadIdx.x; i < nrows; i += kThreads) ys[i] = 0.0;
-  const int wave = threadIdx.x >> 6, lane = threadIdx.x & 63;
+  const int wave = wave_id(), lane = threadIdx.x & 63;
   bool first = true;
   for (int j = 0; j < Gp; j++) {
     const int b = g * Gp + j;
@@ -330,35 +379,43 @@
     first = false;
     int sl = s0 + wave;
     size_t nbase = 0;
-    int nL = 0, nrow = -1;
-    if (sl < s0 + ns) { nbase = (size_t)slice_base[sl]; nL = slice_len[sl]; nrow = slice_rows[(size_t)sl * 64 + lane]; }
+    int nL = 0;
+    uint32_t nw = 0u;
+    if (sl < s0 + ns) { nbase = (size_t)slice_base[sl]; nL = slice_len[sl]; nw = slice_lanes[(size_t)sl * 64 + lane]; }
     for (; sl < s0 + ns; sl += kWaves) {
-      const size_t base = nbase + lane;
-      const int L = nL, row = nrow;
+      const double *v = sval + nbase;
+      const ColT *c = scol + nbase;
+      const int L = nL, len = lane_len(nw), row = (int)(nw & 4095u);
       if (sl + kWaves < s0 + ns) {
-        nbase = (size_t)slice_base[sl + kWaves]; nL = slice_len[sl + kWaves]; nrow = slice_rows[(size_t)(sl + kWaves) * 64 + lane];
+        nbase = (size_t)slice_base[sl + kWaves]; nL = slice_len[sl + kWaves]; nw = slice_lanes[(size_t)(sl + kWaves) * 64 + lane];
       }
-      const double *v = sval + base;
-      const ColT *c = scol + base;
       double a0 = 0.0;
+      uint32_t start = (uint32_t)lane;
       for (int k = 0; k < L; k += kBatch) {
         double cv[kBatch];
         ColT cc[kBatch];
+        uint32_t at[kBatch];
+#pragma unroll
+        for (int u = 0; u < kBatch; u++) { at[u] = start; start += column_lanes(k + u < len, gm); }
         if (k + kBatch <= L) {
 #pragma unroll
-          for (int u = 0; u < kBatch; u++) { cv[u] = v[(size_t)(k + u) * 64]; cc[u] = c[(size_t)(k + u) * 64]; }
+          for (int u = 0; u < kBatch; u++) { cv[u] = slice_at(v, at[u]); cc[u] = slice_at(c, at[u]); }
         } else {
 #pragma unroll
           for (int u = 0; u < kBatch; u++) {
             const bool in = k + u < L;
-            cv[u] = in ? v[(size_t)(k + u) * 64] : 0.0;
-            cc[u] = in ? c[(size_t)(k + u) * 64] : (ColT)0;
+            cv[u] = in ? slice_at(v, at[u]) : 0.0;
+            cc[u] = in ? slice_at(c, at[u]) : (ColT)0;
           }
         }
 #pragma unroll
-        for (int u = 0; u < kBatch; u++) a0 += (kSquare ? cv[u] * cv[u] : cv[u]) * xs[cc[u]];
+        for (int u = 0; u < kBatch; u++) {
+          const bool mine = k + u < len;
+          const double val = mine ? cv[u] : 0.0;
+          a0 += (kSquare ? val * val : val) * xs[mine ? cc[u] : (ColT)0];
+        }
       }
-      if (row >= 0) ys[row - r0] += a0;
+      if (len > 0) ys[row] += a0;
     }
   }
   __syncthreads();
@@ -366,21 +423,21 @@
   for (int i = threadIdx.x; i < nrows; i += kThreads) out[i] = ys[i];
 }
 template <typename ColT, bool kStageX, bool kSquare = false>
-__global__ __launch_bounds__(kThreads) void k_spmv_sell(int rows, int cols, int shift, int B, int Gp, const int *__restrict__ tile_g,
+__global__ __launch_bounds__(kThreads) void k_spmv_sell(int rows, int cols, int shift, int gm, int B, int Gp, const int *__restrict__ tile_g,
                                                         const int *__restrict__ tile_r0, const int *__restrict__ tile_r1,
                                                         const int *__restrict__ unit_s0, const int *__restrict__ unit_ns,
                                                         const uint32_t *__restrict__ slice_base, const int *__restrict__ slice_len,
-                                                        const int *__restrict__ slice_rows, const ColT *__restrict__ scol,
+                                                        const uint32_t *__restrict__ slice_lanes, const ColT *__restrict__ scol,
                                                         const double *__restrict__ sval, const double *__restrict__ x,
                                                         double *__restrict__ partial, const int *__restrict__ skip) {
   if (skip && *skip) return;
-  sell_tile<ColT, kStageX, kSquare>(blockIdx.x, rows, cols, shift, B, Gp, tile_g, tile_r0, tile_r1, unit_s0, unit_ns, slice_base, slice_len,
-                                    slice_rows, scol, sval, x, partial);
+  sell_tile<ColT, kStageX, kSquare>(blockIdx.x, rows, cols, shift, gm, B, Gp, tile_g, tile_r0, tile_r1, unit_s0, unit_ns, slice_base, slice_len,
+                                    slice_lanes, scol, sval, x, partial);
 }
 struct SellSide {
-  int rows, cols, B, Gp, ntiles;
-  const int *tile_g, *tile_r0, *tile_r1, *unit_s0, *unit_ns, *slice_len, *slice_rows;
-  const uint32_t *slice_base;
+  int rows, cols, B, Gp, ntiles, gm;
+  const int *tile_g, *tile_r0, *tile_r1, *unit_s0, *unit_ns, *slice_len;
+  const uint32_t *slice_base, *slice_lanes;
   const uint16_t *scol;
   const double *sval;
   double *partial;
@@ -390,8 +447,8 @@
   if (skip && *skip) return;
   const bool first = (int)blockIdx.x < a.ntiles;
   const SellSide &m = first ? a : b;
-  sell_tile<uint16_t, true, false>(first ? (int)blockIdx.x : (int)blockIdx.x - a.ntiles, m.rows, m.cols, shift, m.B, m.Gp, m.tile_g, m.tile_r0,
-                                   m.tile_r1, m.unit_s0, m.unit_ns, m.slice_base, m.slice_len, m.slice_rows, m.scol, m.sval, x, m.partial);
+  sell_tile<uint16_t, true, false>(first ? (int)blockIdx.x : (int)blockIdx.x - a.ntiles, m.rows, m.cols, shift, m.gm, m.B, m.Gp, m.tile_g, m.tile_r0,
+                                   m.tile_r1, m.unit_s0, m.unit_ns, m.slice_base, m.slice_len, m.slice_lanes, m.scol, m.sval, x, m.partial);
 }
 
 __device__ __forceinline__ void panel_reduce_rows(int vb, int vg, int rows, int B, const double *__restrict__ partial, double *__restrict__ y,
@@ -470,11 +527,11 @@
 }
 
 template <typename ColT, int kOp>
-__global__ __launch_bounds__(kThreads) void k_sell_visit(int rows, int shift, int B, int Gp, const int *__restrict__ tile_g,
+__global__ __launch_bounds__(kThreads) void k_sell_visit(int rows, int shift, int gm, int B, int Gp, const int *__restrict__ tile_g,
                                                          const int *__restrict__ tile_r0, const int *__restrict__ tile_r1,
                                                          const int *__restrict__ unit_s0, const int *__restrict__ unit_ns,
                                                          const uint32_t *__restrict__ slice_base, const int *__restrict__ slice_len,
-                                                         const int *__restrict__ slice_rows, const ColT *__restrict__ scol,
+                                                         const uint32_t *__restrict__ slice_lanes, const ColT *__restrict__ scol,
                                                          double *__restrict__ sval, const double *__restrict__ r, const double *__restrict__ c,
                                                          int order, double scalar, int row0, double *__restrict__ out) {
   __shared__ double ys[kOp == 1 ? kTileRowsMax : 1];
@@ -491,11 +548,14 @@
     for (int sl = s0 + wave; sl < s0 + ns; sl += kWaves) {
       const size_t base = (size_t)slice_base[sl] + lane;
       const int L = slice_len[sl];
-      const int row = slice_rows[(size_t)sl * 64 + lane];
-      if (row < 0) continue;
+      const uint32_t w = slice_lanes[(size_t)sl * 64 + lane];
+      const int row = lane_row(w, r0), len = lane_len(w);
       double mx = 0.0;
+      uint32_t start = 0u;
       for (int k = 0; k < L; k++) {
-        const size_t at = base + (size_t)k * 64;
+        const size_t at = base + start;
+        start += column_lanes(k < len, gm);
+        if (k >= len) continue;
         double v = sval[at];
         if (kOp == 0) {
           if (r) {
@@ -514,7 +574,7 @@
           if (c0 + (int)scol[at] == row + row0 && v != 0.0) out[row] = v;
         }
       }
-      if (kOp == 1) ys[row - r0] = fmax(ys[row - r0], mx);
+      if (kOp == 1 && len > 0) ys[row - r0] = fmax(ys[row - r0], mx);
     }
   }
   if (kOp == 1) {
@@ -524,11 +584,11 @@
   }
 }
 template <typename ColT>
-__global__ __launch_bounds__(kThreads) void k_sell_scale_norm(int rows, int cols, int shift, int B, int Gp, const int *__restrict__ tile_g,
+__global__ __launch_bounds__(kThreads) void k_sell_scale_norm(int rows, int cols, int shift, int gm, int B, int Gp, const int *__restrict__ tile_g,
                                                               const int *__restrict__ tile_r0, const int *__restrict__ tile_r1,
                                                               const int *__restrict__ unit_s0, const int *__restrict__ unit_ns,
                                                               const uint32_t *__restrict__ slice_base, const int *__restrict__ slice_len,
-                                                              const int *__restrict__ slice_rows, const ColT *__restrict__ scol,
+                                                              const uint32_t *__restrict__ slice_lanes, const ColT *__restrict__ scol,
                                                               double *__restrict__ sval, const double *__restrict__ r,
                                                               const double *__restrict__ c, int order, double pre, int row0,
                                                               double *__restrict__ partial) {
@@ -538,7 +598,7 @@
   const int r0 = tile_r0[t], nrows = tile_r1[t] - r0;
   double *cs = lds, *ys = lds + W;
   for (int i = threadIdx.x; i < nrows; i += kThreads) ys[i] = 0.0;
-  const int wave = threadIdx.x >> 6, lane = threadIdx.x & 63;
+  const int wave = wave_id(), lane = threadIdx.x & 63;
   const double *rv = order == 1 ? c + row0 : r;
   bool first = true;
   for (int j = 0; j < Gp; j++) {
@@ -566,39 +626,46 @@
     size_t nbase = 0;
     int nL = 0, nrow = -1;
     double nrs = 1.0;
+    uint32_t nw = 0u;
     if (sl < s0 + ns) {
-      nbase = (size_t)slice_base[sl]; nL = slice_len[sl]; nrow = slice_rows[(size_t)sl * 64 + lane];
+      nbase = (size_t)slice_base[sl]; nL = slice_len[sl]; nw = slice_lanes[(size_t)sl * 64 + lane];
+      nrow = lane_row(nw, r0);
       nrs = nrow >= 0 ? rv[nrow] : 1.0;
     }
     for (; sl < s0 + ns; sl += kWaves) {
-      const size_t base = nbase + lane;
-      const int L = nL, row = nrow;
+      double *v = sval + nbase;
+      const ColT *cc_ = scol + nbase;
+      const int L = nL, row = nrow, len = lane_len(nw);
       const double rs = nrs;
       if (sl + kWaves < s0 + ns) {
-        nbase = (size_t)slice_base[sl + kWaves]; nL = slice_len[sl + kWaves]; nrow = slice_rows[(size_t)(sl + kWaves) * 64 + lane];
+        nbase = (size_t)slice_base[sl + kWaves]; nL = slice_len[sl + kWaves]; nw = slice_lanes[(size_t)(sl + kWaves) * 64 + lane];
+        nrow = lane_row(nw, r0);
         nrs = nrow >= 0 ? rv[nrow] : 1.0;
       }
-      double *v = sval + base;
-      const ColT *cc_ = scol + base;
       const int grow = row + row0 - c0;
       double mx = 0.0;
+      uint32_t start = (uint32_t)lane;
       for (int k = 0; k < L; k += kBatch) {
         double cv[kBatch];
         ColT cc[kBatch];
+        uint32_t at[kBatch];
+#pragma unroll
+        for (int u = 0; u < kBatch; u++) { at[u] = start; start += column_lanes(k + u < len, gm); }
         const bool full = k + kBatch <= L;
         if (full) {
 #pragma unroll
-          for (int u = 0; u < kBatch; u++) { cv[u] = v[(size_t)(k + u) * 64]; cc[u] = cc_[(size_t)(k + u) * 64]; }
+          for (int u = 0; u < kBatch; u++) { cv[u] = slice_at(v, at[u]); cc[u] = slice_at(cc_, at[u]); }
         } else {
 #pragma unroll
           for (int u = 0; u < kBatch; u++) {
             const bool in = k + u < L;
-            cv[u] = in ? v[(size_t)(k + u) * 64] : 0.0;
-            cc[u] = in ? cc_[(size_t)(k + u) * 64] : (ColT)0;
+            cv[u] = in ? slice_at(v, at[u]) : 0.0;
+            cc[u] = in ? slice_at(cc_, at[u]) : (ColT)0;
           }
         }
 #pragma unroll
         for (int u = 0; u < kBatch; u++) {
+          if (k + u >= len) { cv[u] = 0.0; cc[u] = (ColT)0; }
           double x = cv[u];
           if (pre != 1.0) x *= pre;
           const double cf = cs[cc[u]];
@@ -608,15 +675,8 @@
           cv[u] = x;
           mx = fmax(mx, fabs(x));
         }
-        if (row >= 0) {
-          if (full) {
-#pragma unroll
-            for (int u = 0; u < kBatch; u++) v[(size_t)(k + u) * 64] = cv[u];
-          } else {
-#pragma unroll
-            for (int u = 0; u < kBatch; u++) if (k + u < L) v[(size_t)(k + u) * 64] = cv[u];
-          }
-        }
+#pragma unroll
+        for (int u = 0; u < kBatch; u++) if (k + u < len) slice_at(v, at[u]) = cv[u];
       }
       if (row >= 0) ys[row - r0] = fmax(ys[row - r0], mx);
     }
@@ -634,7 +694,9 @@
   out[i] = accumulate ? fmax(out[i], m) : m;
 }
 __global__ __launch_bounds__(kBlock) void k_sell_slot_of_pos(int rows, int shift, const int64_t *__restrict__ rp, const int *__restrict__ col,
-                                                             const uint32_t *__restrict__ cellbase, uint32_t *__restrict__ slot) {
+                                                             const uint32_t *__restrict__ cellbase, const uint32_t *__restrict__ slice_base,
+                                                             const uint32_t *__restrict__ slice_tab, const uint32_t *__restrict__ colstart,
+                                                             uint32_t *__restrict__ slot) {
   const int lane = threadIdx.x & 63;
   const int64_t row = ((int64_t)blockIdx.x * kBlock + threadIdx.x) >> 6;
   if (row >= rows) return;
@@ -642,7 +704,7 @@
   for (int64_t k = s + lane; k < e; k += 64) {
     const int b = col[k] >> shift;
     const int64_t seg = lower_bound_col(col, s, k + 1, b << shift);
-    slot[k] = (uint32_t)((size_t)cellbase[(size_t)b * rows + row] + (size_t)(k - seg) * 64);
+    slot[k] = (uint32_t)cell_slot(cellbase[(size_t)b * rows + row], k - seg, slice_base, slice_tab, colstart);
   }
 }
 
@@ -695,10 +757,12 @@
   DevPanel &P = M.panel;
   if (P.wide)
     OQ_LAUNCH(k_sell_scatter<uint32_t>, dim3(blocks_for((int64_t)M.rows * 64)), dim3(kBlock), 0, s, M.rows, P.shift, M.rowptr.get(),
-              M.col.get(), M.val.get(), P.cellbase.get(), P.scol32.get(), P.sval.get(), with_cols ? 1 : 0, slot);
+              M.col.get(), M.val.get(), P.cellbase.get(), P.slice_base.get(), P.slice_tab.get(), P.colstart.get(), P.scol32.get(), P.sval.get(),
+              with_cols ? 1 : 0, slot);
   else
     OQ_LAUNCH(k_sell_scatter<uint16_t>, dim3(blocks_for((int64_t)M.rows * 64)), dim3(kBlock), 0, s, M.rows, P.shift, M.rowptr.get(),
-              M.col.get(), M.val.get(), P.cellbase.get(), P.scol.get(), P.sval.get(), with_cols ? 1 : 0, slot);
+              M.col.get(), M.val.get(), P.cellbase.get(), P.slice_base.get(), P.slice_tab.get(), P.colstart.get(), P.scol.get(), P.sval.get(),
+              with_cols ? 1 : 0, slot);
 }
 
 void panel_build(DevCsr &M, hipStream_t s, uint32_t *slot, bool will_compact, const std::function<void()> &after_cols) {
@@ -707,6 +771,8 @@
   P.shift = P.wide ? (wide_shift(M) ? wide_shift(M) : 18) : panel_shift(); P.W = 1 << P.shift;
   if (!P.wide && P.shift > 15) throw PanelRefused(6, "panel width above 2^15 columns is not supported (16-bit local column ids, LDS size)");
   P.B = (M.cols + P.W - 1) >> P.shift;
+  P.align = sell_align();
+  const int gm = P.align - 1;
   const int64_t cells = (int64_t)P.B * M.rows;
   DevBuf<int64_t> cnt((size_t)cells + 1), off((size_t)cells + 1);
   DevBuf<uint32_t> cellsrc((size_t)cells);
@@ -745,48 +811,61 @@
   HIP_CHECK(hipStreamSynchronize(s));
   gcnt.release(); tid.release();
   DevBuf<int64_t> nsl((size_t)nunits + 1), pad((size_t)nunits + 1), slice0((size_t)nunits + 1), padded0((size_t)nunits + 1);
-  OQ_LAUNCH(k_tile_measure, dim3((unsigned)nunits), dim3(kThreads), 0, s, M.rows, ub.get(), u0.get(), u1.get(), off.get(), nsl.get(), pad.get());
+  DevBuf<int64_t> lens((size_t)nunits + 1), lensum0((size_t)nunits + 1);
+  OQ_LAUNCH(k_tile_measure, dim3((unsigned)nunits), dim3(kThreads), 0, s, M.rows, P.align, ub.get(), u0.get(), u1.get(), off.get(), nsl.get(),
+            pad.get(), lens.get());
   exclusive_scan(nsl.get(), slice0.get(), nunits, s);
   exclusive_scan(pad.get(), padded0.get(), nunits, s);
+  exclusive_scan(lens.get(), lensum0.get(), nunits, s);
   const int64_t nslices = read_i64(slice0.get() + nunits, s), padded = read_i64(padded0.get() + nunits, s);
-  if (padded >= 4294967295LL) throw PanelRefused(6, "sliced-ELL copy exceeds 2^32 entries");
-  if (!getenv("OSQP_AMD_PANEL") && (double)padded > 1.5 * (double)M.nnz) throw PanelRefused(6, "sliced-ELL copy would be mostly padding");
+  const int64_t lensum = read_i64(lensum0.get() + nunits, s), padded64 = 64 * lensum;
+  nsl.release(); pad.release(); lens.release();
+  if (padded + kSlack >= 4294967295LL) throw PanelRefused(6, "sliced-ELL copy exceeds 2^32 entries");
+  if (nslices >= (1LL << 26)) throw PanelRefused(6, "sliced-ELL copy exceeds 2^26 slices");
+  if (!getenv("OSQP_AMD_PANEL") && (double)padded64 > 1.5 * (double)M.nnz) throw PanelRefused(6, "sliced-ELL copy would be mostly padding");
   P.padded = (size_t)padded;
   P.unit_s0.alloc((size_t)nunits); P.unit_ns.alloc((size_t)nunits);
-  P.slice_base.alloc((size_t)nslices); P.slice_len.alloc((size_t)nslices); P.slice_rows.alloc((size_t)nslices * 64);
+  P.slice_base.alloc((size_t)nslices); P.slice_len.alloc((size_t)nslices); P.slice_lanes.alloc((size_t)nslices * 64);
   P.cellbase.alloc((size_t)cells); P.cellbase.zero(s);
-  OQ_LAUNCH(k_tile_layout, dim3((unsigned)nunits), dim3(kThreads), 0, s, M.rows, ub.get(), u0.get(), u1.get(), off.get(), slice0.get(),
-            padded0.get(), P.unit_s0.get(), P.unit_ns.get(), P.slice_base.get(), P.slice_len.get(), P.slice_rows.get(), P.cellbase.get());
+  P.slice_tab.alloc((size_t)nslices); P.colstart.alloc((size_t)lensum + 1);
+  OQ_LAUNCH(k_tile_layout, dim3((unsigned)nunits), dim3(kThreads), 0, s, M.rows, P.align, ub.get(), u0.get(), u1.get(), off.get(), slice0.get(),
+            padded0.get(), lensum0.get(), P.unit_s0.get(), P.unit_ns.get(), P.slice_base.get(), P.slice_len.get(), P.slice_lanes.get(),
+            P.cellbase.get(), P.slice_tab.get(), P.colstart.get());
   P.partial.alloc((size_t)gcells);
   P.partial.zero(s);
   static const bool lds_fill = !(getenv("OSQP_AMD_SELL_FILL") && atoi(getenv("OSQP_AMD_SELL_FILL")) == 0);
   auto fill = [&](int what) {
     if (P.wide)
-      OQ_LAUNCH(k_sell_fill_lds<uint32_t>, dim3((unsigned)nunits), dim3(kFillWaves * 64), 0, s, M.rows, P.shift, ub.get(), P.unit_s0.get(),
-                P.unit_ns.get(), P.slice_base.get(), P.slice_len.get(), P.slice_rows.get(), cellsrc.get(), off.get(), M.col.get(), M.val.get(),
-                P.scol32.get(), P.sval.get(), slot, what);
+      OQ_LAUNCH(k_sell_fill_lds<uint32_t>, dim3((unsigned)nunits), dim3(kFillWaves * 64), 0, s, M.rows, P.shift, gm, ub.get(), u0.get(),
+                P.unit_s0.get(), P.unit_ns.get(), P.slice_base.get(), P.slice_len.get(), P.slice_lanes.get(), cellsrc.get(), M.col.get(),
+                M.val.get(), P.scol32.get(), P.sval.get(), slot, what);
     else
-      OQ_LAUNCH(k_sell_fill_lds<uint16_t>, dim3((unsigned)nunits), dim3(kFillWaves * 64), 0, s, M.rows, P.shift, ub.get(), P.unit_s0.get(),
-                P.unit_ns.get(), P.slice_base.get(), P.slice_len.get(), P.slice_rows.get(), cellsrc.get(), off.get(), M.col.get(), M.val.get(),
-                P.scol.get(), P.sval.get(), slot, what);
+      OQ_LAUNCH(k_sell_fill_lds<uint16_t>, dim3((unsigned)nunits), dim3(kFillWaves * 64), 0, s, M.rows, P.shift, gm, ub.get(), u0.get(),
+                P.unit_s0.get(), P.unit_ns.get(), P.slice_base.get(), P.slice_len.get(), P.slice_lanes.get(), cellsrc.get(), M.col.get(),
+                M.val.get(), P.scol.get(), P.sval.get(), slot, what);
+  };
+  auto alloc_vals = [&] { P.sval.alloc((size_t)padded + kSlack); HIP_CHECK(hipMemsetAsync(P.sval.get() + padded, 0, sizeof(double) * kSlack, s)); };
+  auto alloc_cols = [&] {
+    if (P.wide) { P.scol32.alloc((size_t)padded + kSlack); HIP_CHECK(hipMemsetAsync(P.scol32.get() + padded, 0, sizeof(uint32_t) * kSlack, s)); }
+    else { P.scol.alloc((size_t)padded + kSlack); HIP_CHECK(hipMemsetAsync(P.scol.get() + padded, 0, sizeof(uint16_t) * kSlack, s)); }
   };
   if (!lds_fill) {
-    P.sval.alloc((size_t)padded);
+    P.sval.alloc((size_t)padded + kSlack);
     P.sval.zero(s);
-    if (P.wide) { P.scol32.alloc((size_t)padded); P.scol32.zero(s); }
-    else { P.scol.alloc((size_t)padded); P.scol.zero(s); }
+    if (P.wide) { P.scol32.alloc((size_t)padded + kSlack); P.scol32.zero(s); }
+    else { P.scol.alloc((size_t)padded + kSlack); P.scol.zero(s); }
     panel_fill(M, true, s, slot);
   } else if (will_compact && !P.wide) {
-    P.scol.alloc((size_t)padded);
+    alloc_cols();
     fill(1);
     HIP_CHECK(hipStreamSynchronize(s));
     M.col.release();
     if (after_cols) after_cols();
-    P.sval.alloc((size_t)padded);
+    alloc_vals();
     fill(2);
   } else {
-    P.sval.alloc((size_t)padded);
-    if (P.wide) P.scol32.alloc((size_t)padded); else P.scol.alloc((size_t)padded);
+    alloc_vals();
+    alloc_cols();
     fill(3);
   }
   HIP_CHECK(hipStreamSynchronize(s));
@@ -803,13 +882,13 @@
   const DevPanel &P = M.panel;
   const SpmvExtra ex = extra ? *extra : SpmvExtra();
   if (P.wide)
-    OQ_LAUNCH((k_spmv_sell<uint32_t, false>), dim3(P.ntiles), dim3(kThreads), sizeof(double) * kTileRowsMax, s, M.rows, M.cols, P.shift, P.B,
-              P.Gp, P.tile_g.get(), P.tile_r0.get(), P.tile_r1.get(), P.unit_s0.get(), P.unit_ns.get(), P.slice_base.get(),
-              P.slice_len.get(), P.slice_rows.get(), P.scol32.get(), P.sval.get(), x, P.partial.get(), g_skip);
+    OQ_LAUNCH((k_spmv_sell<uint32_t, false>), dim3(P.ntiles), dim3(kThreads), sizeof(double) * kTileRowsMax, s, M.rows, M.cols, P.shift, P.align - 1,
+              P.B, P.Gp, P.tile_g.get(), P.tile_r0.get(), P.tile_r1.get(), P.unit_s0.get(), P.unit_ns.get(), P.slice_base.get(),
+              P.slice_len.get(), P.slice_lanes.get(), P.scol32.get(), P.sval.get(), x, P.partial.get(), g_skip);
   else
-    OQ_LAUNCH((k_spmv_sell<uint16_t, true>), dim3(P.ntiles), dim3(kThreads), spmv_lds_bytes(P.shift), s, M.rows, M.cols, P.shift, P.B,
-              P.Gp, P.tile_g.get(), P.tile_r0.get(), P.tile_r1.get(), P.unit_s0.get(), P.unit_ns.get(), P.slice_base.get(),
-              P.slice_len.get(), P.slice_rows.get(), P.scol.get(), P.sval.get(), x, P.partial.get(), g_skip);
+    OQ_LAUNCH((k_spmv_sell<uint16_t, true>), dim3(P.ntiles), dim3(kThreads), spmv_lds_bytes(P.shift), s, M.rows, M.cols, P.shift, P.align - 1,
+              P.B, P.Gp, P.tile_g.get(), P.tile_r0.get(), P.tile_r1.get(), P.unit_s0.get(), P.unit_ns.get(), P.slice_base.get(),
+              P.slice_len.get(), P.slice_lanes.get(), P.scol.get(), P.sval.get(), x, P.partial.get(), g_skip);
   OQ_LAUNCH(k_panel_reduce, dim3(reduce_grid(M.rows)), dim3(kBlock), 0, s, M.rows, P.NG, P.partial.get(), y, rscale, beta, gamma, v, ex, g_skip);
 }
 
@@ -823,9 +902,9 @@
   auto side = [](const DevCsr &M) {
     const DevPanel &P = M.panel;
     SellSide t;
-    t.rows = M.rows; t.cols = M.cols; t.B = P.B; t.Gp = P.Gp; t.ntiles = P.ntiles;
+    t.rows = M.rows; t.cols = M.cols; t.B = P.B; t.Gp = P.Gp; t.ntiles = P.ntiles; t.gm = P.align - 1;
     t.tile_g = P.tile_g.get(); t.tile_r0 = P.tile_r0.get(); t.tile_r1 = P.tile_r1.get(); t.unit_s0 = P.unit_s0.get(); t.unit_ns = P.unit_ns.get();
-    t.slice_len = P.slice_len.get(); t.slice_rows = P.slice_rows.get(); t.slice_base = P.slice_base.get(); t.scol = P.scol.get();
+    t.slice_len = P.slice_len.get(); t.slice_lanes = P.slice_lanes.get(); t.slice_base = P.slice_base.get(); t.scol = P.scol.get();
     t.sval = P.sval.get(); t.partial = P.partial.get();
     return t;
   };
@@ -843,12 +922,12 @@
 
 #define OQ_SELL_VISIT(OP, ...)                                                                                                              \
   do {                                                                                                                                      \
-    if (P.wide) OQ_LAUNCH((k_sell_visit<uint32_t, OP>), dim3(P.ntiles), dim3(kThreads), 0, s, M.rows, P.shift, P.B, P.Gp, P.tile_g.get(),    \
+    if (P.wide) OQ_LAUNCH((k_sell_visit<uint32_t, OP>), dim3(P.ntiles), dim3(kThreads), 0, s, M.rows, P.shift, P.align - 1, P.B, P.Gp, P.tile_g.get(), \
                           P.tile_r0.get(), P.tile_r1.get(), P.unit_s0.get(), P.unit_ns.get(), P.slice_base.get(), P.slice_len.get(),        \
-                          P.slice_rows.get(), P.scol32.get(), P.sval.get(), __VA_ARGS__);                                                    \
-    else OQ_LAUNCH((k_sell_visit<uint16_t, OP>), dim3(P.ntiles), dim3(kThreads), 0, s, M.rows, P.shift, P.B, P.Gp, P.tile_g.get(),           \
+                          P.slice_lanes.get(), P.scol32.get(), P.sval.get(), __VA_ARGS__);                                                    \
+    else OQ_LAUNCH((k_sell_visit<uint16_t, OP>), dim3(P.ntiles), dim3(kThreads), 0, s, M.rows, P.shift, P.align - 1, P.B, P.Gp, P.tile_g.get(), \
                    P.tile_r0.get(), P.tile_r1.get(), P.unit_s0.get(), P.unit_ns.get(), P.slice_base.get(), P.slice_len.get(),               \
-                   P.slice_rows.get(), P.scol.get(), P.sval.get(), __VA_ARGS__);                                                             \
+                   P.slice_lanes.get(), P.scol.get(), P.sval.get(), __VA_ARGS__);                                                             \
   } while (0)
 
 void panel_row_absmax(const DevCsr &M, double *out, bool accumulate, hipStream_t s) {
@@ -865,9 +944,9 @@
   if (P.wide) throw Error(6, "internal: the fused scaling pass needs LDS-staged panels");
   HIP_CHECK(hipFuncSetAttribute((const void *)k_sell_scale_norm<uint16_t>, hipFuncAttributeMaxDynamicSharedMemorySize,
                                 (int)spmv_lds_bytes(P.shift)));
-  OQ_LAUNCH((k_sell_scale_norm<uint16_t>), dim3(P.ntiles), dim3(kThreads), spmv_lds_bytes(P.shift), s, M.rows, M.cols, P.shift, P.B, P.Gp,
-            P.tile_g.get(), P.tile_r0.get(), P.tile_r1.get(), P.unit_s0.get(), P.unit_ns.get(), P.slice_base.get(), P.slice_len.get(),
-            P.slice_rows.get(), P.scol.get(), P.sval.get(), r, c, order, pre, row0, P.partial.get());
+  OQ_LAUNCH((k_sell_scale_norm<uint16_t>), dim3(P.ntiles), dim3(kThreads), spmv_lds_bytes(P.shift), s, M.rows, M.cols, P.shift, P.align - 1, P.B,
+            P.Gp, P.tile_g.get(), P.tile_r0.get(), P.tile_r1.get(), P.unit_s0.get(), P.unit_ns.get(), P.slice_base.get(), P.slice_len.get(),
+            P.slice_lanes.get(), P.scol.get(), P.sval.get(), r, c, order, pre, row0, P.partial.get());
   OQ_LAUNCH(k_panel_reduce_max, dim3(blocks_for(M.rows)), dim3(kBlock), 0, s, M.rows, P.NG, P.partial.get(), norm, 0);
 }
 void panel_diag(const DevCsr &M, double *diag, int row0, hipStream_t s) {
@@ -880,22 +959,24 @@
   const DevPanel &P = M.panel;
   HIP_CHECK(hipFuncSetAttribute((const void *)k_spmv_sell<uint16_t, true, true>, hipFuncAttributeMaxDynamicSharedMemorySize,
                                 (int)spmv_lds_bytes(P.shift)));
-  OQ_LAUNCH((k_spmv_sell<uint16_t, true, true>), dim3(P.ntiles), dim3(kThreads), spmv_lds_bytes(P.shift), s, M.rows, M.cols, P.shift, P.B,
-            P.Gp, P.tile_g.get(), P.tile_r0.get(), P.tile_r1.get(), P.unit_s0.get(), P.unit_ns.get(), P.slice_base.get(),
-            P.slice_len.get(), P.slice_rows.get(), P.scol.get(), P.sval.get(), x, P.partial.get(), (const int *)nullptr);
+  OQ_LAUNCH((k_spmv_sell<uint16_t, true, true>), dim3(P.ntiles), dim3(kThreads), spmv_lds_bytes(P.shift), s, M.rows, M.cols, P.shift, P.align - 1,
+            P.B, P.Gp, P.tile_g.get(), P.tile_r0.get(), P.tile_r1.get(), P.unit_s0.get(), P.unit_ns.get(), P.slice_base.get(),
+            P.slice_len.get(), P.slice_lanes.get(), P.scol.get(), P.sval.get(), x, P.partial.get(), (const int *)nullptr);
   OQ_LAUNCH(k_panel_reduce, dim3(reduce_grid(M.rows)), dim3(kBlock), 0, s, M.rows, P.NG, P.partial.get(), y, (const double *)nullptr, 0.0, gamma, v,
             SpmvExtra(), (const int *)nullptr);
 }
 void panel_slot_of_pos(const DevCsr &M, uint32_t *slot, hipStream_t s) {
   const DevPanel &P = M.panel;
   OQ_LAUNCH(k_sell_slot_of_pos, dim3(blocks_for((int64_t)M.rows * 64)), dim3(kBlock), 0, s, M.rows, P.shift, M.rowptr.get(), M.col.get(),
-            P.cellbase.get(), slot);
+            P.cellbase.get(), P.slice_base.get(), P.slice_tab.get(), P.colstart.get(), slot);
 }
 bool panel_can_compact(const DevCsr &M) { return M.panel.active && !M.panel.wide; }
 void panel_compact(DevCsr &M) {
   M.col.release();
   M.val.release();
   M.panel.cellbase.release();
+  M.panel.slice_tab.release();
+  M.panel.colstart.release();
   M.compact = true;
 }
 
```

Measured after the change: 75.33 iterations/s. 0.903x the previous value.
